# hsinnan75/Kart

Measured on AMD Instinct MI355X. Metric: mapped reads/sec (whole node), 150 bp PE, higher is better.
Workload: dtype u64

## Files before the change

kart_amd/csrc/abi.hip:

```cpp
#include "abi_internal.hpp"
#include <cmath>

#include <algorithm>
#include <atomic>
#include <cstdarg>
#include <cstdio>
#include <cstdlib>
#include <cstring>
#include <memory>
#include <mutex>
#include <string>
#include <thread>
#include <vector>

namespace kg { KG_INTERNAL thread_local KernelTimer *kt_current = nullptr; }

namespace {

thread_local char g_err[512] = "";

}

int kg_fail(int code, const char *fmt, ...)
{
// ... 98 lines not shown
		if (v.seq_len == 0 || v.primary > v.seq_len || (uint64_t)n_words < need)
			return fail(KG_ERR_IO, "%s.bwt is truncated or malformed (%llu words for %llu symbols, need %llu)", prefix, (unsigned long long)n_words,
			            (unsigned long long)v.seq_len, (unsigned long long)need);
	}
	uint64_t sa_intv = 0, sa_len = 0;
	memcpy(&sa_intv, sa.data() + 40, 8);
	memcpy(&sa_len, sa.data() + 48, 8);
	if (sa_intv != 32) return fail(KG_ERR_IO, "%s.sa: unsupported SA interval %llu (expected 32)", prefix, (unsigned long long)sa_intv);
	if (sa_len != v.seq_len) return fail(KG_ERR_IO, "%s: .sa and .bwt disagree on the sequence length", prefix);
	ix->n_sa = (v.seq_len + 32) / 32;
	if ((sa.size() - 56) / 8 < ix->n_sa - 1) return fail(KG_ERR_IO, "%s.sa is truncated", prefix);

	{
		FILE *fp = fopen((pre + ".ann").c_str(), "r");
		if (!fp) return fail(KG_ERR_IO, "cannot read %s.ann", prefix);
		long long l_pac = 0;
		int n_seqs = 0;
		unsigned seed = 0;
		if (fscanf(fp, "%lld%d%u", &l_pac, &n_seqs, &seed) != 3) { fclose(fp); return fail(KG_ERR_IO, "%s.ann: bad header", prefix); }
		ix->l_pac = l_pac;
		int64_t total = 0;
		for (int i = 0; i < n_seqs; ++i) {
			unsigned gi;
			char name[1024];
			long long off;
			int len, n_ambs, ch;
			if (fscanf(fp, "%u%1023s", &gi, name) != 2) { fclose(fp); return fail(KG_ERR_IO, "%s.ann: bad contig record %d", prefix, i); }
			while ((ch = fgetc(fp)) != '\n' && ch != EOF) {}
			if (fscanf(fp, "%lld%d%d", &off, &len, &n_ambs) != 3) { fclose(fp); return fail(KG_ERR_IO, "%s.ann: bad contig record %d", prefix, i); }
			ContigRec c;
			c.name = name;
			c.len = len;
			c.fwd_start = total;
			total += len;
			c.rev_start = 2 * ix->l_pac - total;
			ix->contigs.push_back(c);
		}
		fclose(fp);
		if ((uint64_t)(2 * ix->l_pac) != v.seq_len) return fail(KG_ERR_IO, "%s: .ann l_pac does not match the BWT length", prefix);
	}
	size_t pac_bytes = (size_t)(ix->l_pac / 4 + 1);
	if (pac.size() < pac_bytes) return fail(KG_ERR_IO, "%s.pac is truncated", prefix);
	ix->pac.assign(pac.data(), pac.data() + pac_bytes);

	size_t occ_bytes = n_words * 4 + 128;
	HIP_TRY(hipMalloc((void **)&ix->d_occ, occ_bytes));
	HIP_TRY(hipMemset(ix->d_occ, 0, occ_bytes));
	HIP_TRY(hipMemcpy(ix->d_occ, bwt.data() + 40, n_words * 4, hipMemcpyHostToDevice));
	const uint64_t sa0 = (uint64_t)-1;
	HIP_TRY(hipMalloc((void **)&ix->d_sa, ix->n_sa * 8));
	HIP_TRY(hipMemcpy(ix->d_sa, &sa0, 8, hipMemcpyHostToDevice));
	if (ix->n_sa > 1) HIP_TRY(hipMemcpy(ix->d_sa + 1, sa.data() + 56, (ix->n_sa - 1) * 8, hipMemcpyHostToDevice));
	HIP_TRY(hipMalloc((void **)&ix->d_pac, pac_bytes));
	HIP_TRY(hipMemcpy(ix->d_pac, ix->pac.data(), pac_bytes, hipMemcpyHostToDevice));
	{
		std::vector<std::pair<int64_t, int32_t>> ec;
		for (size_t i = 0; i < ix->contigs.size(); ++i) {
			const ContigRec &c = ix->contigs[i];
			ec.emplace_back(c.fwd_start + c.len - 1, (int32_t)i);
			ec.emplace_back(c.rev_start + c.len - 1, (int32_t)i);
		}
		std::sort(ec.begin(), ec.end());
		std::vector<int64_t> ends;
		std::vector<int32_t> echr;
		for (const std::pair<int64_t, int32_t> &e : ec) { ends.push_back(e.first); echr.push_back(e.second); }
		ix->n_ends = (int)ends.size();
		HIP_TRY(hipMalloc((void **)&ix->d_contig_end, 8 * ends.size() + 8));
		HIP_TRY(hipMemcpy(ix->d_contig_end, ends.data(), 8 * ends.size(), hipMemcpyHostToDevice));
		HIP_TRY(hipMalloc((void **)&ix->d_end_chr, 4 * echr.size() + 8));
		HIP_TRY(hipMemcpy(ix->d_end_chr, echr.data(), 4 * echr.size(), hipMemcpyHostToDevice));
		std::vector<int64_t> tab;
		for (const ContigRec &c : ix->contigs) tab.push_back(c.fwd_start);
		for (const ContigRec &c : ix->contigs) tab.push_back(c.rev_start);
		for (const ContigRec &c : ix->contigs) tab.push_back(c.len);
		HIP_TRY(hipMalloc((void **)&ix->d_chr_tab, 8 * tab.size() + 8));
		HIP_TRY(hipMemcpy(ix->d_chr_tab, tab.data(), 8 * tab.size(), hipMemcpyHostToDevice));
		std::vector<uint8_t> mq((size_t)(kAlnMaxScore + 1) * 6 + (size_t)(kAlnMaxScore + 1) * 8, 0);
		for (int sc = 1; sc <= kAlnMaxScore; ++sc)
			for (int d = 1; d <= 5 && d < sc; ++d) {
				int sub = sc - d;
				int q = (int)(30 * (1 - (float)(sc - sub) / sc) * log(sc) + 0.4999);
				mq[(size_t)sc * 6 + (size_t)d] = (uint8_t)(q > 60 ? 60 : q < 0 ? 0 : q);
			}
		for (int sc = 1; sc < 8; ++sc)
			for (int nd = 1; nd <= kAlnMaxScore; ++nd) {
				int sub = sc + nd;
				int q = (int)(30 * (1 - (float)(sc - sub) / sc) * log(sc) + 0.4999);
				mq[(size_t)(kAlnMaxScore + 1) * 6 + (size_t)sc * (kAlnMaxScore + 1) + (size_t)nd] = (uint8_t)(q > 60 ? 60 : q < 0 ? 0 : q);
			}
		HIP_TRY(hipMalloc((void **)&ix->d_mapq_tab, mq.size()));
		HIP_TRY(hipMemcpy(ix->d_mapq_tab, mq.data(), mq.size(), hipMemcpyHostToDevice));
	}
	ix->device_bytes = occ_bytes + ix->n_sa * 8 + pac_bytes;
	v.occ = ix->d_occ;
	v.sa = ix->d_sa;
	{
		uint64_t n_blocks64 = ((v.seq_len + 127) / 128) * 2;
		size_t plane_bytes = (size_t)n_blocks64 * 64 + 64;
		HIP_TRY(hipMalloc((void **)&ix->d_planes, plane_bytes));
		HIP_TRY(launch_build_planes(ix->d_occ, n_blocks64, ix->d_planes, nullptr));
		HIP_TRY(hipDeviceSynchronize());
		v.planes = ix->d_planes;
		ix->device_bytes += plane_bytes;
	}
	v.planes2 = nullptr;
	v.planes3 = nullptr;
	for (int i = 0; i < 16; ++i) v.t2[i] = 0;
	for (int i = 0; i < 64; ++i) v.t3[i] = 0;
	if (!getenv("KG_NO_PLANES2")) {
		uint64_t n_lines = (v.seq_len + kPlane2Rows - 1) / kPlane2Rows;
		size_t bytes = (size_t)n_lines * 16 * 128;
		uint64_t *t_dev = nullptr;
		if (hipMalloc((void **)&ix->d_planes2, bytes) == hipSuccess) {
			HIP_TRY(hipMalloc((void **)&t_dev, (16 + 64) * 8));
			HIP_TRY(launch_build_planes_k(v, 2, ix->d_planes2, n_lines, t_dev, t_dev + 16, nullptr));
			HIP_TRY(hipMemcpy(v.t2, t_dev, 16 * 8, hipMemcpyDeviceToHost));
			HIP_TRY(hipMemcpy(v.t3, t_dev + 16, 64 * 8, hipMemcpyDeviceToHost));
			HIP_TRY(hipFree(t_dev));
			v.planes2 = ix->d_planes2;
			ix->device_bytes += bytes;
		} else (void)hipGetLastError();
	}
	v.fsa32 = nullptr;
	v.fsa64 = nullptr;
	v.fsa40 = nullptr;
	v.dsa32 = nullptr;
	v.dsa64 = nullptr;
	v.dsa_shift = 0;
	v.text = nullptr;
	{
		size_t text_bytes = (size_t)(v.seq_len / 4 + 1) + 16;
		HIP_TRY(hipMalloc((void **)&ix->d_text, text_bytes));
		HIP_TRY(launch_build_text(ix->d_pac, (uint64_t)ix->l_pac, ix->d_text, text_bytes, nullptr));
		HIP_TRY(hipDeviceSynchronize());
		ix->device_bytes += text_bytes;
	}
	v.qtab32 = nullptr;
	v.qtab64 = nullptr;
	v.qmer = 0;

	const bool dense = sa_mode == KG_SA_DENSE4 || sa_mode == KG_SA_DENSE8;
	const bool wide = sa_mode == KG_SA_FULL40_WIDE;
	const bool compact = sa_mode == KG_SA_FULL40 || wide;
	if (sa_mode == KG_SA_FULL || dense || compact) {
		bool narrow = v.seq_len < 0xFFFFFFFFull && !getenv("KG_FORCE_U64");
		const bool packed = compact && !narrow;
		if (packed && v.seq_len >= (1ull << 40)) return fail(KG_ERR_ARG, "kg_index_load: KG_SA_FULL40 holds texts below 2^40 bases");
		size_t fsa_bytes = packed ? (size_t)(v.seq_len + 1) * 5 + 8 : (size_t)(v.seq_len + 1) * (narrow ? 4 : 8);
		HIP_TRY(hipMalloc(&ix->d_fsa, fsa_bytes));
		uint32_t *f32 = narrow ? (uint32_t *)ix->d_fsa : nullptr;
		uint64_t *f64 = narrow || packed ? nullptr : (uint64_t *)ix->d_fsa;
		uint8_t *f40 = packed ? (uint8_t *)ix->d_fsa : nullptr;
		HIP_TRY(launch_expand_sa(v, ix->n_sa, f32, f64, f40, nullptr));
		HIP_TRY(hipDeviceSynchronize());
		v.fsa32 = f32;
		v.fsa64 = f64;
		v.fsa40 = f40;
		if (!dense) ix->device_bytes += fsa_bytes;
		if (!getenv("KG_NO_DIRECT")) v.text = ix->d_text;
	} else if (sa_mode != KG_SA_SAMPLED) {
		return fail(KG_ERR_ARG, "kg_index_load: unknown sa_mode %d", sa_mode);
	}
	if (!getenv("KG_NO_QTAB")) {
		bool narrow = v.seq_len < 0xFFFFFF00ull && !getenv("KG_FORCE_U64");
		int q = kQmerMin;
		while (q < kQmerMax && ((uint64_t)1 << (2 * q + 1)) <= v.seq_len) q++;
		if (compact && !wide && q > kQmerMin) q--;
		if (const char *env = getenv("KG_QMER")) { int t = atoi(env); if (t >= kQmerMin && t <= kQmerMax) q = t; }
		size_t tab_bytes = ((size_t)1 << (2 * q)) * 8;
		while (hipMalloc(&ix->d_qtab, tab_bytes) != hipSuccess) {
			(void)hipGetLastError();
			ix->d_qtab = nullptr;
			if (q <= kQmerMin) return fail(KG_ERR_NOMEM, "kg_index_load: no device memory for the q-mer table");
			q--;
			tab_bytes >>= 2;
		}
		v.qmer = q;
		HIP_TRY(launch_build_qtab(v, q, narrow ? (uint2 *)ix->d_qtab : nullptr, narrow ? nullptr : (uint64_t *)ix->d_qtab, nullptr));
		HIP_TRY(hipDeviceSynchronize());
		if (narrow) v.qtab32 = (const uint2 *)ix->d_qtab; else v.qtab64 = (const uint64_t *)ix->d_qtab;
		ix->device_bytes += tab_bytes;
	}
	if (dense) {
		const int shift = sa_mode == KG_SA_DENSE4 ? 2 : 3;
		const bool narrow = v.fsa32 != nullptr;
		const uint64_t n_out = (v.seq_len >> shift) + 1;
		const size_t bytes = (size_t)n_out * (narrow ? 4 : 8);
		HIP_TRY(hipMalloc(&ix->d_dsa, bytes));
		HIP_TRY(launch_sample_sa(v.fsa32, v.fsa64, n_out, shift, narrow ? (uint32_t *)ix->d_dsa : nullptr, narrow ? nullptr : (uint64_t *)ix->d_dsa, nullptr));
		HIP_TRY(hipDeviceSynchronize());
		HIP_TRY(hipFree(ix->d_fsa));
		ix->d_fsa = nullptr;
		v.fsa32 = nullptr; v.fsa64 = nullptr;
		if (narrow) v.dsa32 = (const uint32_t *)ix->d_dsa; else v.dsa64 = (const uint64_t *)ix->d_dsa;
		v.dsa_shift = shift;
		ix->device_bytes += bytes;
	}
	if (v.planes2 && !dense && (!compact || wide) && !getenv("KG_NO_PLANES3")) {
		uint64_t n_lines = (v.seq_len + kPlane2Rows - 1) / kPlane2Rows;
		size_t bytes = (size_t)n_lines * 64 * 128, free_b = 0, total_b = 0;
		const size_t reserve = (size_t)48 << 30;
		if (hipMemGetInfo(&free_b, &total_b) == hipSuccess && free_b > bytes + reserve && hipMalloc((void **)&ix->d_planes3, bytes) == hipSuccess) {
			HIP_TRY(launch_build_planes_k(v, 3, ix->d_planes3, n_lines, nullptr, nullptr, nullptr));
			v.planes3 = ix->d_planes3;
			ix->device_bytes += bytes;
		} else (void)hipGetLastError();
	}
	*out = ix.release();
	return KG_OK;
}

void kg_index_destroy(kg_index *ix)
{
	if (!ix) return;
	(void)hipSetDevice(ix->device);
	kgi_frag_release(ix);
	if (ix->d_occ) (void)hipFree(ix->d_occ);
	if (ix->d_planes) (void)hipFree(ix->d_planes);
	if (ix->d_planes2) (void)hipFree(ix->d_planes2);
	if (ix->d_planes3) (void)hipFree(ix->d_planes3);
	if (ix->d_qtab) (void)hipFree(ix->d_qtab);
	for (NwScratch *sc : ix->nw_pool) {
		if (sc->done) { (void)hipEventSynchronize(sc->done); (void)hipEventDestroy(sc->done); }
		if (sc->lists) (void)hipFree(sc->lists);
		if (sc->queue) (void)hipFree(sc->queue);
		if (sc->dir) (void)hipFree(sc->dir);
		if (sc->io) (void)hipFree(sc->io);
		if (sc->io_stream) (void)hipStreamDestroy(sc->io_stream);
		delete sc;
	}
	if (ix->d_sa) (void)hipFree(ix->d_sa);
	if (ix->d_fsa) (void)hipFree(ix->d_fsa);
	if (ix->d_dsa) (void)hipFree(ix->d_dsa);
	if (ix->d_text) (void)hipFree(ix->d_text);
	if (ix->d_pac) (void)hipFree(ix->d_pac);
	if (ix->d_contig_end) (void)hipFree(ix->d_contig_end);
	if (ix->d_end_chr) (void)hipFree(ix->d_end_chr);
	if (ix->d_chr_tab) (void)hipFree(ix->d_chr_tab);
	if (ix->d_mapq_tab) (void)hipFree(ix->d_mapq_tab);
	delete ix;
}

int kg_index_info(const kg_index *ix, kg_index_info_t *info)
{
	if (!ix || !info) return fail(KG_ERR_ARG, "kg_index_info: null argument");
	info->genome_size = ix->l_pac;
	info->seq_len = ix->view.seq_len;
	info->primary = ix->view.primary;
	info->n_contigs = (int32_t)ix->contigs.size();
	int k = 13;
	for (; k < 16; ++k)
		if ((double)(2 * ix->l_pac) < (double)(1ull << (2 * k))) break;
	info->min_seed_len = k;
	info->sa_mode = ix->sa_mode;
	info->device = ix->device;
	info->device_bytes = ix->device_bytes;
	return KG_OK;
}

int kg_index_contig(const kg_index *ix, int i, kg_contig_t *out)
{
	if (!ix || !out || i < 0 || i >= (int)ix->contigs.size()) return fail(KG_ERR_ARG, "kg_index_contig: bad argument");
	const ContigRec &c = ix->contigs[(size_t)i];
	out->name = c.name.c_str();
	out->fwd_start = c.fwd_start;
	out->rev_start = c.rev_start;
	out->len = c.len;
	return KG_OK;
}

int kg_rank_sa_batch(kg_index *ix, const uint64_t *k, int64_t n, uint64_t *occ4, uint64_t *sa_walk, uint64_t *sa_full)
{
	if (!ix || !k || n < 0) return fail(KG_ERR_ARG, "kg_rank_sa_batch: bad argument");
	if (n == 0) return KG_OK;
	HIP_TRY(hipSetDevice(ix->device));
	uint64_t *d = nullptr;
	HIP_TRY(hipMalloc((void **)&d, 8 * (size_t)n * 7));
	uint64_t *d_k = d, *d_occ = d + n, *d_walk = d + 5 * n, *d_full = d + 6 * n;
	hipError_t e = hipMemcpy(d_k, k, 8 * (size_t)n, hipMemcpyHostToDevice);
	if (e == hipSuccess) e = launch_rank_sa(ix->view, d_k, n, occ4 ? d_occ : nullptr, sa_walk ? d_walk : nullptr, sa_full ? d_full : nullptr, nullptr);
	if (e == hipSuccess) e = hipDeviceSynchronize();
	if (e == hipSuccess && occ4) e = hipMemcpy(occ4, d_occ, 32 * (size_t)n, hipMemcpyDeviceToHost);
	if (e == hipSuccess && sa_walk) e = hipMemcpy(sa_walk, d_walk, 8 * (size_t)n, hipMemcpyDeviceToHost);
	if (e == hipSuccess && sa_full) e = hipMemcpy(sa_full, d_full, 8 * (size_t)n, hipMemcpyDeviceToHost);
	(void)hipFree(d);
	if (e != hipSuccess) return fail(KG_ERR_NO_DEVICE, "kg_rank_sa_batch: %s", hipGetErrorString(e));
	return KG_OK;
}

void *kg_host_alloc(size_t bytes)
{
	void *p = nullptr;
	if (hipHostMalloc(&p, bytes ? bytes : 1, hipHostMallocPortable) != hipSuccess) { (void)hipGetLastError(); return nullptr; }
	return p;
}

void kg_host_free(void *p)
{
	if (p) (void)hipHostFree(p);
}

int kg_workspace_create(kg_index *ix, int64_t max_reads, int64_t max_bases, kg_workspace **out)
{
	if (!ix || !out || max_reads <= 0 || max_bases <= 0) return fail(KG_ERR_ARG, "kg_workspace_create: bad argument");
	*out = nullptr;
	HIP_TRY(hipSetDevice(ix->device));
	std::unique_ptr<kg_workspace, void (*)(kg_workspace *)> ws(new kg_workspace(), kg_workspace_destroy);
	ws->ix = ix;
	ws->max_reads = max_reads;
	ws->max_bases = max_bases;
	ws->max_hits = max_bases / 13 + max_bases / 52 + max_reads + (int64_t)ix->n_cu * 32 * 256 + 4096;
	HIP_TRY(hipMalloc((void **)&ws->d_hits, sizeof(Hit) * (size_t)ws->max_hits));
	HIP_TRY(hipMalloc((void **)&ws->d_packed, 8 * (size_t)(max_bases / 16 + 3 * max_reads + 64)));
	HIP_TRY(hipMalloc((void **)&ws->d_seeds_per_read, 4 * (size_t)max_reads));
	HIP_TRY(hipMalloc((void **)&ws->d_ctl, 8 * kCtlWords));
	ws->scan_bytes = scan_temp_bytes(max_reads + 1);
	HIP_TRY(hipMalloc(&ws->d_scan_temp, ws->scan_bytes ? ws->scan_bytes : 256));
	if (getenv("KG_SORT_READS")) {
		ws->sort_bytes = sort_temp_bytes(max_reads);
		HIP_TRY(hipMalloc((void **)&ws->d_sort_keys, 16 * (size_t)max_reads + 64));
		HIP_TRY(hipMalloc(&ws->d_sort_temp, ws->sort_bytes ? ws->sort_bytes : 256));
	}
	HIP_TRY(hipStreamCreateWithFlags(&ws->stream, hipStreamNonBlocking));
	HIP_TRY(hipMemsetAsync(ws->d_ctl, 0, 8 * kCtlWords, ws->stream));
	HIP_TRY(hipHostMalloc((void **)&ws->h_small, 8 * 16, hipHostMallocDefault));
	*out = ws.release();
	return KG_OK;
}

void kg_workspace_destroy(kg_workspace *ws)
{
	if (!ws) return;
	(void)hipSetDevice(ws->ix->device);
	if (ws->stream) { (void)hipStreamSynchronize(ws->stream); (void)hipStreamDestroy(ws->stream); }
	kgi_long_release(ws);
	for (int i = 0; i < kg_workspace::kRing; ++i) {
		if (ws->ring_cands[i]) (void)hipHostFree(ws->ring_cands[i]);
		if (ws->ring_seeds[i]) (void)hipHostFree(ws->ring_seeds[i]);
		if (ws->ring_records[i]) (void)hipHostFree(ws->ring_records[i]);
	}
	void *ptrs[] = {ws->d_sort_keys, ws->d_sort_temp, ws->d_plans, ws->d_tasks, ws->d_aln_cand, ws->d_aln_read, ws->d_spill, ws->d_jobs, ws->d_job_ops, ws->d_job_len, ws->d_chunk_off, ws->d_chunk_paired, ws->d_chunk_stats, ws->d_aln_ctl, ws->d_used, ws->d_cand_off, ws->d_cseed_off, ws->d_dense_cands, ws->d_dense_seeds, ws->d_cands, ws->d_cand_seeds, ws->d_n_cands, ws->d_taken, ws->d_hits, ws->d_packed, ws->d_seeds_per_read, ws->d_ctl, ws->d_scan_temp, ws->d_enc, ws->d_read_off, ws->d_seed_off, ws->d_seeds, ws->d_vr_n, ws->d_vr_off, ws->d_vr_read, ws->d_vr_pos, ws->d_claim, ws->d_step};
	for (void *p : ptrs)
		if (p) (void)hipFree(p);
	if (ws->h_seeds) (void)hipHostFree(ws->h_seeds);
	if (ws->h_small) (void)hipHostFree(ws->h_small);
	if (ws->sync_ev) (void)hipEventDestroy(ws->sync_ev);
	for (hipEvent_t e : ws->ev)
		if (e) (void)hipEventDestroy(e);
	for (int i = 0; i < KT_SLOTS; ++i) {
		for (int j = 0; j < kKtRing; ++j) {
			if (ws->kt.b[i][j]) (void)hipEventDestroy(ws->kt.b[i][j]);
			if (ws->kt.e[i][j]) (void)hipEventDestroy(ws->kt.e[i][j]);
		}
	}
	delete ws;
}

int kg_workspace_counters(kg_workspace *ws, kg_counters_t *out)
{
	if (!ws || !out) return fail(KG_ERR_ARG, "kg_workspace_counters: null argument");
	HIP_TRY(hipSetDevice(ws->ix->device));
	HIP_TRY(hipDeviceSynchronize());
	unsigned long long ctl[kCtlWords];
	HIP_TRY(hipMemcpy(ctl, ws->d_ctl, sizeof(ctl), hipMemcpyDeviceToHost));
	out->searches = ctl[4]; out->lf1 = ctl[5]; out->lf2 = ctl[6]; out->inv = ctl[7];
	out->sa = ctl[8]; out->seeds = ctl[9]; out->bases = ctl[10];
	return KG_OK;
}

int kg_workspace_traffic(kg_workspace *ws, kg_traffic_t *out)
{
	if (!ws || !out) return fail(KG_ERR_ARG, "kg_workspace_traffic: null argument");
	HIP_TRY(hipSetDevice(ws->ix->device));
	HIP_TRY(hipDeviceSynchronize());
	unsigned long long ctl[kCtlWords];
	HIP_TRY(hipMemcpy(ctl, ws->d_ctl, sizeof(ctl), hipMemcpyDeviceToHost));
	out->table_lookups = ctl[17]; out->rank_steps = ctl[18]; out->rank_steps_two_lines = ctl[19];
	out->text_rounds = ctl[20]; out->window_words = ctl[21]; out->rank_steps_two_lines_narrow = ctl[22];
	out->sa_gathers = ctl[8]; out->hits = ctl[1]; out->searches = ctl[4];
	out->sa_entry_bytes = (ws->ix->view.fsa32 ? 4 : ws->ix->view.fsa40 ? 5 : 8);
	out->double_steps = ctl[23]; out->double_steps_two_lines = ctl[24]; out->double_step_bytes = ctl[25]; out->triple_steps = ctl[26];
	return KG_OK;
}

int kg_workspace_set_single_steps(kg_workspace *ws, int enabled)
{
	if (!ws) return fail(KG_ERR_ARG, "kg_workspace_set_single_steps: null workspace");
	ws->single_steps = enabled != 0;
	return KG_OK;
}

int kg_index_selfcheck(kg_index *ix, int64_t samples, uint64_t seed, uint64_t *disagreements)
{
	if (!ix || !disagreements || samples < 0) return fail(KG_ERR_ARG, "kg_index_selfcheck: bad argument");
	*disagreements = 0;
	if (!ix->view.planes2) return fail(KG_ERR_ARG, "kg_index_selfcheck: the index holds no two-step rank structure");
	HIP_TRY(hipSetDevice(ix->device));
	unsigned long long *bad = nullptr;
	HIP_TRY(hipMalloc((void **)&bad, 8));
	HIP_TRY(hipMemset(bad, 0, 8));
	HIP_TRY(hipDeviceSynchronize());
	hipError_t e = launch_planes2_check(ix->view, (uint64_t)samples, seed, bad, nullptr);
	unsigned long long h = 0;
	hipError_t e2 = hipMemcpy(&h, bad, 8, hipMemcpyDeviceToHost);
	(void)hipFree(bad);
	if (e != hipSuccess || e2 != hipSuccess) return fail(KG_ERR_NO_DEVICE, "kg_index_selfcheck: %s", hipGetErrorString(e != hipSuccess ? e : e2));
	*disagreements = h;
	return KG_OK;
}

int kg_workspace_set_profiling(kg_workspace *ws, int enabled)
{
	if (!ws) return fail(KG_ERR_ARG, "kg_workspace_set_profiling: null workspace");
	HIP_TRY(hipSetDevice(ws->ix->device));
	if (enabled && !ws->ev[0])
		for (int i = 0; i < 5; ++i) HIP_TRY(hipEventCreate(&ws->ev[i]));
	if (enabled && !ws->kt.b[0][0])
		for (int i = 0; i < KT_SLOTS; ++i)
			for (int j = 0; j < kKtRing; ++j) { HIP_TRY(hipEventCreate(&ws->kt.b[i][j])); HIP_TRY(hipEventCreate(&ws->kt.e[i][j])); }
	ws->profiling = enabled != 0;
	return KG_OK;
}

int kg_workspace_kernel_ms(kg_workspace *ws, float ms[4])
{
	if (!ws || !ms) return fail(KG_ERR_ARG, "kg_workspace_kernel_ms: null argument");
	if (!ws->profiling || !ws->ev[0]) return fail(KG_ERR_ARG, "kg_workspace_kernel_ms: profiling is not enabled");
	HIP_TRY(hipSetDevice(ws->ix->device));
	HIP_TRY(hipEventSynchronize(ws->ev[4]));
	for (int i = 0; i < 4; ++i) HIP_TRY(hipEventElapsedTime(&ms[i], ws->ev[i], ws->ev[i + 1]));
	return KG_OK;
}

int64_t kg_workspace_overflow(kg_workspace *ws)
{
	if (!ws) return -1;
	if (hipSetDevice(ws->ix->device) != hipSuccess || hipDeviceSynchronize() != hipSuccess) return -1;
	unsigned long long v = 0;
	if (hipMemcpy(&v, ws->d_ctl + 11, 8, hipMemcpyDeviceToHost) != hipSuccess) return -1;
	return (int64_t)v;
}

int64_t kg_workspace_segment_fallbacks(kg_workspace *ws)
{
	return ws ? ws->segment_fallbacks : -1;
}

static int check_seed_args(kg_workspace *ws, int mode, int min_seed_len, int occ_thr, int64_t n_reads, int64_t n_bases)
{
	if (!ws) return fail(KG_ERR_ARG, "kg_seed_batch: null workspace");
	if ((mode & ~KG_INPUT_ASCII) != KG_MODE_FAST && (mode & ~KG_INPUT_ASCII) != KG_MODE_SENSITIVE) return fail(KG_ERR_ARG, "kg_seed_batch: unknown mode %d", mode);
	if (min_seed_len < 13 || min_seed_len > 16) return fail(KG_ERR_ARG, "kg_seed_batch: min_seed_len %d outside 13..16", min_seed_len);
	if (occ_thr < 1 || occ_thr > 1000000) return fail(KG_ERR_ARG, "kg_seed_batch: occ_thr %d out of range", occ_thr);
	if (n_reads < 0 || n_reads > ws->max_reads) return fail(KG_ERR_CAPACITY, "kg_seed_batch: %lld reads exceed the workspace (%lld)", (long long)n_reads, (long long)ws->max_reads);
	if (n_bases < 0 || n_bases > ws->max_bases) return fail(KG_ERR_CAPACITY, "kg_seed_batch: %lld bases exceed the workspace (%lld)", (long long)n_bases, (long long)ws->max_bases);
	return KG_OK;
}

int kg_seed_batch_device(kg_workspace *ws, int mode, int min_seed_len, int occ_thr, const uint8_t *d_enc_bases,
                         const int64_t *d_read_offsets, int64_t n_reads, int64_t n_bases, int64_t *d_seed_offsets,
                         kg_seed *d_seeds, int64_t seed_capacity, void *stream)
{
	int rc = check_seed_args(ws, mode, min_seed_len, occ_thr, n_reads, n_bases);
	if (rc != KG_OK) return rc;
	if (!d_read_offsets || !d_seed_offsets || (n_bases > 0 && !d_enc_bases) || (seed_capacity > 0 && !d_seeds) || seed_capacity < 0)
		return fail(KG_ERR_ARG, "kg_seed_batch_device: null buffer");
	HIP_TRY(hipSetDevice(ws->ix->device));
	hipStream_t st = (hipStream_t)stream;
	if (n_reads == 0) {
		HIP_TRY(hipMemsetAsync(d_seed_offsets, 0, 8, st));
		return KG_OK;
	}
	SeedArgs a;
	a.ix = ws->ix->view;
	a.enc = d_enc_bases;
	a.read_off = d_read_offsets;
	a.n_reads = n_reads;
	a.n_bases = n_bases;
	a.mode = mode & ~KG_INPUT_ASCII;
	a.ascii = (mode & KG_INPUT_ASCII) ? 1 : 0;
	a.min_seed_len = min_seed_len;
	a.occ_thr = occ_thr;
	a.packed = ws->d_packed;
	a.single_steps = ws->single_steps ? 1 : 0;
	a.read_order = nullptr; a.sort_keys = ws->d_sort_keys; a.sort_temp = ws->d_sort_temp; a.sort_temp_bytes = ws->sort_bytes;
	a.hits = ws->d_hits;
	a.max_hits = ws->max_hits;
	a.seeds_per_read = ws->d_seeds_per_read;
	a.read_queue = ws->d_ctl + 0;
	a.hit_count = ws->d_ctl + 1;
	a.locate_queue = ws->d_ctl + 2;
	a.counters = ws->d_ctl + 4;
	a.traffic = ws->d_ctl + 17;
	a.seed_off = d_seed_offsets;
	a.seeds = d_seeds;
	a.seed_capacity = seed_capacity;
	a.read_len = nullptr; a.n_seg = 0; a.seg_stride = 0;
	for (int64_t &x : a.seg_prefix) x = 0;
	const bool no_segments = getenv("KG_NO_SEGMENTS") != nullptr;
	const int seg_len = getenv("KG_SEG_LEN") ? std::max(128, atoi(getenv("KG_SEG_LEN"))) : 512;
	ws->last_segmented = false;
	if (a.mode == KG_MODE_SENSITIVE && !no_segments && ws->segments_off_batches == 0 && ws->group_segments == 0 && n_bases >= 4 * (int64_t)seg_len * n_reads) {
		ws->last_segmented = true;
		if (!ws->d_vr_n) {
			ws->vr_capacity = ws->max_bases / 128 + ws->max_reads + 64;
			HIP_TRY(hipMalloc((void **)&ws->d_vr_n, 4 * (size_t)(ws->max_reads + 2)));
			HIP_TRY(hipMalloc((void **)&ws->d_vr_off, 8 * (size_t)(ws->max_reads + 2)));
			HIP_TRY(hipMalloc((void **)&ws->d_vr_read, 4 * (size_t)ws->vr_capacity));
			HIP_TRY(hipMalloc((void **)&ws->d_vr_pos, 4 * (size_t)ws->vr_capacity));
			HIP_TRY(hipMalloc((void **)&ws->d_claim, 4 * (size_t)((ws->max_bases >> 5) + ws->max_reads + 64)));
			HIP_TRY(hipMalloc((void **)&ws->d_step, (size_t)ws->max_bases + 64));
		}
		a.seg_len = seg_len;
		a.vr_read = ws->d_vr_read; a.vr_pos = ws->d_vr_pos;
		a.vr_total = reinterpret_cast<const unsigned long long *>(ws->d_vr_off + n_reads);
		a.claim = ws->d_claim; a.step = ws->d_step;
		HIP_TRY(launch_seed_segments(a, ws->d_vr_n, ws->d_vr_off, ws->d_vr_read, ws->d_vr_pos, ws->d_scan_temp, ws->scan_bytes, ws->ix->n_cu, st));
	}
	if (ws->group_segments > 0) {
		a.read_len = ws->group_read_len;
		a.n_seg = ws->group_segments;
		a.seg_stride = ws->group_stride;
		for (int i = 0; i <= a.n_seg; ++i) a.seg_prefix[i] = ws->group_prefix[i];
	}
	HIP_TRY(launch_seed_batch(a, ws->d_scan_temp, ws->scan_bytes, ws->ix->n_cu, st, ws->profiling ? ws->ev : nullptr));
	return KG_OK;
}

hipError_t kgi_sync(kg_workspace *ws)
{
	static const bool spin = getenv("KG_SPIN_SYNC") != nullptr;
	if (spin) return hipStreamSynchronize(ws->stream);
	if (!ws->sync_ev) {
		hipError_t e = hipEventCreateWithFlags(&ws->sync_ev, hipEventBlockingSync | hipEventDisableTiming);
		if (e != hipSuccess) return e;
	}
	hipError_t e = hipEventRecord(ws->sync_ev, ws->stream);
	if (e != hipSuccess) return e;
	return hipEventSynchronize(ws->sync_ev);
}

int kgi_seed_resident(kg_workspace *ws, int mode, int min_seed_len, int occ_thr, int64_t n_reads, int64_t n_bases, int64_t *total_out)
{
	int rc = check_seed_args(ws, mode, min_seed_len, occ_thr, n_reads, n_bases);
	if (rc != KG_OK) return rc;
	int64_t want = std::max<int64_t>(ws->seed_capacity, 8 * std::max(n_reads, ws->max_reads) + 1024);
	int64_t total = 0;
	bool retried_plain = false;
	for (int attempt = 0; attempt < 2; ++attempt) {
		if (want > ws->seed_capacity) {
			if (ws->d_seeds) HIP_TRY(hipFree(ws->d_seeds));
			ws->d_seeds = nullptr;
			HIP_TRY(hipMalloc((void **)&ws->d_seeds, sizeof(kg_seed) * (size_t)want));
			ws->seed_capacity = want;
		}
		rc = kg_seed_batch_device(ws, mode, min_seed_len, occ_thr, ws->d_enc, ws->d_read_off, n_reads, n_bases,
		                          ws->d_seed_off, ws->d_seeds, ws->seed_capacity, ws->stream);
		if (rc != KG_OK) return rc;
		unsigned long long *h = ws->h_small;
		HIP_TRY(hipMemcpyAsync(&h[0], ws->d_seed_off + n_reads, 8, hipMemcpyDeviceToHost, ws->stream));
		HIP_TRY(hipMemcpyAsync(&h[1], ws->d_ctl + 11, 8, hipMemcpyDeviceToHost, ws->stream));
		HIP_TRY(kgi_sync(ws));
		if (h[1] == (~0ull >> 1)) {
			if (ws->last_segmented && !retried_plain) {
				retried_plain = true;
				ws->segments_off_batches = 17;
				ws->segment_fallbacks++;
				--attempt;
				continue;
			}
			return fail(KG_ERR_CAPACITY, "kg_seed_batch: the hit list of the workspace overflowed");
		}
		total = (int64_t)h[0];
		if (total <= ws->seed_capacity) break;
		want = total;
		if (attempt == 1) return fail(KG_ERR_CAPACITY, "kg_seed_batch: seed buffer overflow persisted");
	}
	if (ws->segments_off_batches > 0) ws->segments_off_batches--;
	ws->last_reads = n_reads;
	ws->last_seeds = total;
	ws->last_cands = -1;
	ws->last_ascii = (mode & KG_INPUT_ASCII) != 0;
	*total_out = total;
	return KG_OK;
}

int kgi_seed_group(kg_workspace *ws, int mode, int min_seed_len, int occ_thr, int n_seg, int64_t stride, const int64_t *counts, int64_t *seed_base)
{
	if (n_seg < 1 || n_seg > kMaxSeedSegments || stride < 1 || (int64_t)n_seg * stride > ws->max_reads) return fail(KG_ERR_ARG, "kgi_seed_group: %d segments of %lld slots do not fit the group's workspace", n_seg, (long long)stride);
	ws->group_segments = n_seg;
	ws->group_stride = stride;
	ws->group_prefix[0] = 0;
	for (int i = 0; i < n_seg; ++i) {
		if (counts[i] < 0 || counts[i] > stride) return fail(KG_ERR_ARG, "kgi_seed_group: segment %d holds %lld reads, its slots are %lld", i, (long long)counts[i], (long long)stride);
		ws->group_prefix[i + 1] = ws->group_prefix[i] + counts[i];
	}
	const int64_t n_slots = (int64_t)n_seg * stride;
	int64_t total = 0;
	int rc = kgi_seed_resident(ws, mode, min_seed_len, occ_thr, n_slots, ws->max_bases, &total);
	if (rc != KG_OK) return rc;
	unsigned long long *h = ws->h_small;
	for (int i = 0; i < n_seg; ++i) HIP_TRY(hipMemcpyAsync(&h[2 + i], ws->d_seed_off + (int64_t)i * stride, 8, hipMemcpyDeviceToHost, ws->stream));
	HIP_TRY(kgi_sync(ws));
	for (int i = 0; i < n_seg; ++i) seed_base[i] = (int64_t)h[2 + i];
	seed_base[n_seg] = total;
	return KG_OK;
}

int kg_seed_batch(kg_workspace *ws, int mode, int min_seed_len, int occ_thr, const uint8_t *enc_bases,
                  const int64_t *read_offsets, int64_t n_reads, int64_t *seed_offsets, const kg_seed **seeds)
{
	if (!ws || !read_offsets || !seed_offsets) return fail(KG_ERR_ARG, "kg_seed_batch: null argument");
	if (seeds) *seeds = nullptr;
	int64_t n_bases = n_reads > 0 ? read_offsets[n_reads] - read_offsets[0] : 0;
	if (n_reads > 0 && read_offsets[0] != 0) return fail(KG_ERR_ARG, "kg_seed_batch: read_offsets[0] must be 0");
	int rc = check_seed_args(ws, mode, min_seed_len, occ_thr, n_reads, n_bases);
	if (rc != KG_OK) return rc;
	if (n_reads == 0) { seed_offsets[0] = 0; return KG_OK; }
	HIP_TRY(hipSetDevice(ws->ix->device));
	if (!ws->d_enc) {
		HIP_TRY(hipMalloc((void **)&ws->d_enc, (size_t)ws->max_bases + 64));
		HIP_TRY(hipMalloc((void **)&ws->d_read_off, 8 * (size_t)(ws->max_reads + 1)));
		HIP_TRY(hipMalloc((void **)&ws->d_seed_off, 8 * (size_t)(ws->max_reads + 1)));
	}
	HIP_TRY(hipMemcpyAsync(ws->d_enc, enc_bases, (size_t)n_bases, hipMemcpyHostToDevice, ws->stream));
	HIP_TRY(hipMemcpyAsync(ws->d_read_off, read_offsets, 8 * (size_t)(n_reads + 1), hipMemcpyHostToDevice, ws->stream));
	int64_t total = 0;
	rc = kgi_seed_resident(ws, mode, min_seed_len, occ_thr, n_reads, n_bases, &total);
	if (rc != KG_OK) return rc;
	HIP_TRY(hipMemcpyAsync(seed_offsets, ws->d_seed_off, 8 * (size_t)(n_reads + 1), hipMemcpyDeviceToHost, ws->stream));
	HIP_TRY(kgi_sync(ws));
	if (!seeds) return KG_OK;
	if (total > ws->h_seed_capacity) {
		if (ws->h_seeds) HIP_TRY(hipHostFree(ws->h_seeds));
		ws->h_seeds = nullptr;
		int64_t cap = std::max<int64_t>(total, ws->seed_capacity);
		HIP_TRY(hipHostMalloc((void **)&ws->h_seeds, sizeof(kg_seed) * (size_t)cap, hipHostMallocDefault));
// ... 481 lines not shown
```

kart_amd/csrc/abi_internal.hpp:

```cpp
#pragma once
#include "seed_kernels.hpp"
#include "align_kernels.hpp"

#include <mutex>
#include <string>
#include <vector>

#define KG_INTERNAL __attribute__((visibility("hidden")))
KG_INTERNAL int kg_fail(int code, const char *fmt, ...);

#define HIP_TRY(expr)                                                                                     \
	do {                                                                                                  \
		hipError_t e_ = (expr);                                                                           \
		if (e_ != hipSuccess) return kg_fail(e_ == hipErrorOutOfMemory ? KG_ERR_NOMEM : KG_ERR_NO_DEVICE, \
		                                     "%s: %s", #expr, hipGetErrorString(e_));                     \
	} while (0)

using namespace kg;

struct ContigRec {
	std::string name;
	int64_t fwd_start, rev_start, len;
};

struct NwScratch {
	int32_t *lists = nullptr;
	size_t list_words = 0;
	unsigned long long *queue = nullptr;
	uint32_t *dir = nullptr;
	size_t dir_words = 0;
	hipEvent_t done = nullptr;
	bool busy = false;
	bool pending = false;
	hipStream_t last_stream = nullptr;
	char *io = nullptr;
	size_t io_bytes = 0;
	bool io_busy = false;
	hipStream_t io_stream = nullptr;
};

struct kg_index {
	std::mutex nw_mu;
	std::vector<NwScratch *> nw_pool;
	int device = 0;
	int n_cu = 256;
	int sa_mode = KG_SA_SAMPLED;
	FmView view{};
	int64_t l_pac = 0;
	uint64_t n_sa = 0;
	std::vector<ContigRec> contigs;
	std::vector<uint8_t> pac;
	uint32_t *d_occ = nullptr;
	uint4 *d_planes = nullptr;
	uint4 *d_planes2 = nullptr;
	uint4 *d_planes3 = nullptr;
	void *d_qtab = nullptr;
	uint64_t *d_sa = nullptr;
	void *d_fsa = nullptr;
	void *d_dsa = nullptr;
	uint8_t *d_text = nullptr;
	uint8_t *d_pac = nullptr;
	int64_t *d_contig_end = nullptr;
	int n_ends = 0;
	int32_t *d_end_chr = nullptr;
	int64_t *d_chr_tab = nullptr;
	uint8_t *d_mapq_tab = nullptr;
	uint64_t device_bytes = 0;
};

struct kg_workspace {
	kg_index *ix = nullptr;
	int64_t max_reads = 0, max_bases = 0, max_hits = 0;
	Hit *d_hits = nullptr;
	uint64_t *d_packed = nullptr;
	int32_t *d_seeds_per_read = nullptr;
	unsigned long long *d_ctl = nullptr;
	void *d_scan_temp = nullptr;
	size_t scan_bytes = 0;
	uint32_t *d_sort_keys = nullptr;
	bool single_steps = false;
	void *d_sort_temp = nullptr;
	size_t sort_bytes = 0;
	uint8_t *d_enc = nullptr;
	int64_t *d_read_off = nullptr;
	int64_t *d_seed_off = nullptr;
	kg_seed *d_seeds = nullptr;
	int64_t seed_capacity = 0;
	int64_t last_reads = 0, last_seeds = 0;
	int group_segments = 0;
	bool last_segmented = false;
	int segments_off_batches = 0;
	int64_t segment_fallbacks = 0;
	int64_t group_stride = 0, group_prefix[kMaxSeedSegments + 1] = {0};
	int32_t *group_read_len = nullptr;
	bool enc_borrowed = false;
	kg_candidate *d_cands = nullptr;
	kg_seed *d_cand_seeds = nullptr;
	int32_t *d_n_cands = nullptr;
	uint8_t *d_taken = nullptr;
	int32_t *d_used = nullptr;
	int64_t *d_cand_off = nullptr, *d_cseed_off = nullptr;
	kg_candidate *d_dense_cands = nullptr, *h_cands = nullptr;
	kg_seed *d_dense_seeds = nullptr, *h_cand_seeds = nullptr;
	int64_t h_cand_capacity = 0;
	static constexpr int kRing = 4;
	kg_candidate *ring_cands[kRing] = {nullptr, nullptr, nullptr, nullptr};
	kg_seed *ring_seeds[kRing] = {nullptr, nullptr, nullptr, nullptr};
	int64_t ring_cand_capacity[kRing] = {0, 0, 0, 0};
	kg_aln_record *ring_records[kRing] = {nullptr, nullptr, nullptr, nullptr};
	int64_t ring_record_capacity[kRing] = {0, 0, 0, 0};
	int ring_at = 0, ring_rec_at = 0;
	int64_t cand_capacity = 0, ncand_capacity = 0;
	kg_seed *h_seeds = nullptr;
	int64_t h_seed_capacity = 0;
	int64_t last_cands = -1;
	int64_t last_cand_seeds = 0;
	bool last_pacbio = false;
	void *lr = nullptr;
	int32_t *d_vr_n = nullptr, *d_vr_read = nullptr, *d_vr_pos = nullptr;
	int64_t *d_vr_off = nullptr;
	uint32_t *d_claim = nullptr;
	uint8_t *d_step = nullptr;
	int64_t vr_capacity = 0;
	bool last_ascii = false;
	void *d_aln_cand = nullptr;
	int64_t aln_cand_capacity = 0;
	void *d_aln_read = nullptr;
	int64_t aln_read_capacity = 0;
	kg_aln_record *h_records = nullptr;
	AlnSpill *d_spill = nullptr;
	NwJobDesc *d_jobs = nullptr;
	uint8_t *d_job_ops = nullptr;
	int32_t *d_job_len = nullptr;
	int64_t spill_capacity = 0, job_capacity = 0, ops_capacity = 0;
	void *d_plans = nullptr;
	void *d_tasks = nullptr;
	int64_t task_capacity = 0;
	int64_t *d_chunk_off = nullptr;
	uint8_t *d_chunk_paired = nullptr;
	kg_chunk_stats *d_chunk_stats = nullptr;
	int chunk_capacity = 0;
	unsigned long long *d_aln_ctl = nullptr;
	hipStream_t stream = nullptr;
	hipEvent_t sync_ev = nullptr;
	unsigned long long *h_small = nullptr;
	bool profiling = false;
	hipEvent_t ev[5] = {nullptr, nullptr, nullptr, nullptr, nullptr};
	KernelTimer kt;
};


extern "C" {
KG_INTERNAL hipError_t kgi_sync(kg_workspace *ws);
KG_INTERNAL int kgi_seed_resident(kg_workspace *ws, int mode, int min_seed_len, int occ_thr, int64_t n_reads, int64_t n_bases, int64_t *total_out);
KG_INTERNAL int kgi_seed_group(kg_workspace *ws, int mode, int min_seed_len, int occ_thr, int n_seg, int64_t stride, const int64_t *counts, int64_t *seed_base);
KG_INTERNAL int kgi_chain_resident(kg_workspace *ws, int pacbio, int max_gaps, int64_t totals[2]);
KG_INTERNAL int kgi_nw_launch(kg_index *ix, NwArgs &a, int64_t max_len, hipStream_t st);
KG_INTERNAL void kgi_long_release(kg_workspace *ws);
KG_INTERNAL void kgi_frag_release(kg_index *ix);
KG_INTERNAL int kgi_align_resident(kg_workspace *ws, const int64_t *chunk_off, const uint8_t *chunk_paired, int n_chunks, int est_distance, int max_insert,
                       int max_gaps, int multi_hit, int unset_flag, int64_t host_record_capacity, AlnArgs &a);
}
```

kart_amd/csrc/abi_stream.hip:

```cpp
#include "abi_internal.hpp"
#include "stream_kernels.hpp"

#include <algorithm>
#include <chrono>
#include <condition_variable>
#include <cstdlib>
#include <cstring>
#include <memory>

#define fail kg_fail

namespace {

struct Lane {
	kg_workspace *ws = nullptr;
	uint8_t *d_text[2] = {nullptr, nullptr};
	int32_t *d_tile[2] = {nullptr, nullptr};
	uint32_t *d_line_end[2] = {nullptr, nullptr};
	uint32_t *d_rec[2] = {nullptr, nullptr};
	uint64_t *d_line_acc[2] = {nullptr, nullptr};
	uint32_t *d_rec_line[2] = {nullptr, nullptr};
	int64_t *d_meta = nullptr;
	int32_t *d_read_len = nullptr;
	void *d_scan = nullptr;
	size_t scan_bytes = 0;
	int32_t *d_sam_len = nullptr, *d_host_list = nullptr;
	int64_t *d_sam_off = nullptr;
	unsigned long long *d_sam_ctl = nullptr;
	uint8_t *d_sam = nullptr;
	int64_t d_sam_capacity = 0;
	char *h_text[2] = {nullptr, nullptr};
	int64_t *h_meta = nullptr;
	char *h_sam = nullptr;
	int64_t h_sam_capacity = 0;
	int64_t *h_sam_off = nullptr, *h_cand_off = nullptr;
	int32_t *h_host_list = nullptr;
	uint32_t *h_rec_hdr[2] = {nullptr, nullptr};
	kg_aln_record *h_records = nullptr;
	int64_t record_capacity = 0;
	kg_chunk_stats *h_chunk_stats = nullptr;
	int64_t chunk_capacity = 0;
	kg_candidate *h_cands = nullptr;
	kg_seed *h_cand_seeds = nullptr;
	int64_t h_cand_capacity = 0;
	unsigned long long *h_ctl = nullptr;
	int64_t mapped_reads = 0;
	const kg_aln_record *d_records = nullptr;
	kg_stream_window win{};
	kg_stream_parsed parsed{};
	bool have_batch = false;
	bool fasta = false;
	hipEvent_t ev[8] = {nullptr, nullptr, nullptr, nullptr, nullptr, nullptr, nullptr, nullptr};
	hipEvent_t ev_parsed = nullptr;
};

struct SeedGroup {
	int first = 0, size = 0;
	int64_t stride = 0, seg_bases = 0;
	kg_workspace *ws = nullptr;
	unsigned long long *h_ctl = nullptr;
	std::mutex mu;
	std::condition_variable cv;
	int64_t round = 0;
	int arrived = 0;
	bool present[kMaxSeedSegments] = {false};
	int absent_rounds[kMaxSeedSegments] = {0};
	int64_t n_reads[kMaxSeedSegments] = {0};
	int rc = KG_OK;
	int64_t seed_base[kMaxSeedSegments + 1] = {0};
	bool aborted = false;
	int order[kMaxSeedSegments] = {0};
	int n_order = 0, turn = 0;
};

struct GroupTurn {
	SeedGroup *sg = nullptr;
	bool held = false;
	bool acquire(SeedGroup &g, int j)
	{
		sg = &g;
		std::unique_lock<std::mutex> lk(g.mu);
		g.cv.wait(lk, [&]() { return g.aborted || (g.turn < g.n_order && g.order[g.turn] == j); });
		held = !g.aborted;
		return held;
	}
	void release()
	{
		if (!held) return;
		held = false;
		std::lock_guard<std::mutex> lk(sg->mu);
		sg->turn++;
		sg->cv.notify_all();
	}
	~GroupTurn() { release(); }
};

}

struct kg_stream {
	kg_index *ix = nullptr;
	kg_stream_config cfg{};
	int64_t text_capacity = 0, line_capacity = 0, rec_capacity = 0;
	std::vector<Lane> lanes;
	std::vector<std::unique_ptr<SeedGroup>> groups;
	uint8_t *d_chr_names = nullptr;
	int32_t *d_chr_name_off = nullptr;
	int min_seed_len = 13;
	int format = KG_STREAM_FORMAT_SAM;
	int input = KG_STREAM_INPUT_FASTQ;
	bool fasta_sized = false;
	std::mutex mu;
	kg_stream_timing_t total{};
};

namespace {

void free_lane(Lane &l)
{
	if (l.ws && l.ws->enc_borrowed) l.ws->d_enc = nullptr;
	if (l.ev_parsed) (void)hipEventDestroy(l.ev_parsed);
	if (l.ws) kg_workspace_destroy(l.ws);
	for (int f = 0; f < 2; ++f) {
		if (l.d_text[f]) (void)hipFree(l.d_text[f]);
		if (l.d_tile[f]) (void)hipFree(l.d_tile[f]);
		if (l.d_line_end[f]) (void)hipFree(l.d_line_end[f]);
		if (l.d_rec[f]) (void)hipFree(l.d_rec[f]);
		if (l.d_line_acc[f]) (void)hipFree(l.d_line_acc[f]);
		if (l.d_rec_line[f]) (void)hipFree(l.d_rec_line[f]);
		if (l.h_text[f]) (void)hipHostFree(l.h_text[f]);
		if (l.h_rec_hdr[f]) (void)hipHostFree(l.h_rec_hdr[f]);
	}
	for (void *p : {(void *)l.d_meta, (void *)l.d_read_len, l.d_scan, (void *)l.d_sam_len, (void *)l.d_host_list, (void *)l.d_sam_off, (void *)l.d_sam_ctl, (void *)l.d_sam})
		if (p) (void)hipFree(p);
	for (void *p : {(void *)l.h_meta, (void *)l.h_sam, (void *)l.h_sam_off, (void *)l.h_cand_off, (void *)l.h_host_list, (void *)l.h_records, (void *)l.h_chunk_stats,
	                (void *)l.h_cands, (void *)l.h_cand_seeds, (void *)l.h_ctl})
		if (p) (void)hipHostFree(p);
	for (hipEvent_t e : l.ev)
		if (e) (void)hipEventDestroy(e);
	l = Lane();
}

FqWindow window_of(const kg_stream *s, const Lane &l, int f)
{
	FqWindow w;
	w.text = l.d_text[f];
	w.begin = l.win.begin[f]; w.end = l.win.end[f]; w.eof = l.win.eof[f];
	w.tile_lines = l.d_tile[f];
	w.line_end = l.d_line_end[f];
	w.line_capacity = s->line_capacity;
	uint32_t *r = l.d_rec[f];
	const size_t c = (size_t)s->rec_capacity;
	w.rec_hdr = r; w.rec_name = r + c; w.rec_seq = r + 2 * c; w.rec_qual = r + 3 * c;
	w.rec_rlen = (int32_t *)(r + 4 * c); w.rec_qlen = (int32_t *)(r + 5 * c);
	w.rec_capacity = s->rec_capacity;
	w.line_acc = l.d_line_acc[f]; w.rec_line = l.d_rec_line[f];
	return w;
}

int64_t out_capacity(const kg_stream_config &cfg, int format)
{
	return 2 * cfg.max_window + (format == KG_STREAM_FORMAT_BAM ? 144 : 64) * cfg.max_reads + 4096;
}

float elapsed(hipEvent_t a, hipEvent_t b)
{
	float ms = 0;
	if (hipEventElapsedTime(&ms, a, b) != hipSuccess) { (void)hipGetLastError(); return 0; }
	return ms;
}

}

extern "C" {

int kg_stream_open(kg_index *ix, const kg_stream_config *cfg, kg_stream **out)
{
	if (!ix || !cfg || !out) return fail(KG_ERR_ARG, "kg_stream_open: null argument");
	*out = nullptr;
	if (cfg->lanes < 1 || cfg->lanes > 16 || cfg->max_reads < 2 || cfg->max_window < 4096 || cfg->max_window > 0xF0000000ll)
		return fail(KG_ERR_ARG, "kg_stream_open: bad configuration (%d lanes, %lld reads, %lld bytes per window)", cfg->lanes, (long long)cfg->max_reads, (long long)cfg->max_window);
	const int group = cfg->seed_group > 1 ? cfg->seed_group : 0;
	if (group && (group > kMaxSeedSegments || cfg->lanes % group != 0))
		return fail(KG_ERR_ARG, "kg_stream_open: seed_group %d must divide the %d lanes and be at most %d", group, cfg->lanes, kMaxSeedSegments);
	if (!ix->d_text) return fail(KG_ERR_ARG, "kg_stream_open: the index holds no text");
	HIP_TRY(hipSetDevice(ix->device));
	std::unique_ptr<kg_stream, void (*)(kg_stream *)> s(new kg_stream(), kg_stream_close);
	s->ix = ix;
	s->cfg = *cfg;
	s->text_capacity = (cfg->max_window + 4096 + 255) & ~255ll;
	s->line_capacity = cfg->max_window / 16 + 4096;
	s->rec_capacity = s->line_capacity / 4 + 1;
	{
		kg_index_info_t info;
		kg_index_info(ix, &info);
		s->min_seed_len = info.min_seed_len;
		std::vector<int32_t> off{0};
		std::string names;
		for (const ContigRec &c : ix->contigs) { names += c.name; off.push_back((int32_t)names.size()); }
		HIP_TRY(hipMalloc((void **)&s->d_chr_names, names.size() + 16));
		HIP_TRY(hipMalloc((void **)&s->d_chr_name_off, 4 * off.size()));
		HIP_TRY(hipMemcpy(s->d_chr_names, names.data(), names.size(), hipMemcpyHostToDevice));
		HIP_TRY(hipMemcpy(s->d_chr_name_off, off.data(), 4 * off.size(), hipMemcpyHostToDevice));
	}
	s->lanes.resize((size_t)cfg->lanes);
	const int64_t n = cfg->max_reads;
	const int64_t seg_bases = (cfg->max_window + 4096 + 64 + 255) & ~255ll;
	for (int g = 0; group && g < cfg->lanes / group; ++g) {
		s->groups.push_back(std::unique_ptr<SeedGroup>(new SeedGroup()));
		SeedGroup *sg = s->groups.back().get();
		sg->first = g * group; sg->size = group;
		sg->stride = n + 8; sg->seg_bases = seg_bases;
		int rc = kg_workspace_create(ix, sg->stride * group, seg_bases * group, &sg->ws);
		if (rc != KG_OK) return rc;
		kg_workspace *gw = sg->ws;
		HIP_TRY(hipMalloc((void **)&gw->d_enc, (size_t)gw->max_bases + 64));
		HIP_TRY(hipMalloc((void **)&gw->d_read_off, 8 * (size_t)(gw->max_reads + 1)));
		HIP_TRY(hipMalloc((void **)&gw->d_seed_off, 8 * (size_t)(gw->max_reads + 1)));
		HIP_TRY(hipMalloc((void **)&gw->group_read_len, 4 * (size_t)(gw->max_reads + 1)));
		HIP_TRY(hipMemsetAsync(gw->d_enc, 'N', (size_t)gw->max_bases + 64, gw->stream));
		HIP_TRY(hipMemsetAsync(gw->d_read_off, 0, 8 * (size_t)(gw->max_reads + 1), gw->stream));
		HIP_TRY(hipMemsetAsync(gw->group_read_len, 0, 4 * (size_t)(gw->max_reads + 1), gw->stream));
		HIP_TRY(hipStreamSynchronize(gw->stream));
		HIP_TRY(hipHostMalloc((void **)&sg->h_ctl, 8 * kCtlWords, hipHostMallocDefault));
		(void)kg_workspace_set_profiling(gw, 1);
	}
	for (size_t li = 0; li < s->lanes.size(); ++li) {
		Lane &l = s->lanes[li];
		int rc = kg_workspace_create(ix, n + 8, cfg->max_window + 4096, &l.ws);
		if (rc != KG_OK) return rc;
		kg_workspace *ws = l.ws;
		if (group) {
			SeedGroup &sg = *s->groups[li / (size_t)group];
			ws->d_enc = sg.ws->d_enc + (int64_t)(li % (size_t)group) * sg.seg_bases;
			ws->enc_borrowed = true;
			HIP_TRY(hipEventCreateWithFlags(&l.ev_parsed, hipEventDisableTiming));
		} else
		HIP_TRY(hipMalloc((void **)&ws->d_enc, (size_t)ws->max_bases + 64));
		HIP_TRY(hipMalloc((void **)&ws->d_read_off, 8 * (size_t)(ws->max_reads + 1)));
		HIP_TRY(hipMalloc((void **)&ws->d_seed_off, 8 * (size_t)(ws->max_reads + 1)));
		(void)kg_workspace_set_profiling(ws, 1);
		const int64_t n_tiles = s->text_capacity / kFqTile + 2;
		for (int f = 0; f < 2; ++f) {
			HIP_TRY(hipMalloc((void **)&l.d_text[f], (size_t)s->text_capacity));
			HIP_TRY(hipMalloc((void **)&l.d_tile[f], 4 * (size_t)(n_tiles + 1)));
			HIP_TRY(hipMalloc((void **)&l.d_line_end[f], 4 * (size_t)s->line_capacity));
			HIP_TRY(hipMalloc((void **)&l.d_rec[f], 4 * 6 * (size_t)s->rec_capacity));
			HIP_TRY(hipHostMalloc((void **)&l.h_text[f], (size_t)s->text_capacity, hipHostMallocDefault));
			HIP_TRY(hipHostMalloc((void **)&l.h_rec_hdr[f], 4 * (size_t)(n + 8), hipHostMallocDefault));
		}
		HIP_TRY(hipMalloc((void **)&l.d_meta, 8 * FQM_WORDS));
		HIP_TRY(hipMalloc((void **)&l.d_read_len, 4 * (size_t)(n + 8)));
		l.scan_bytes = fq_scan_temp_bytes(std::max<int64_t>(n + 8, n_tiles + 1));
		HIP_TRY(hipMalloc(&l.d_scan, l.scan_bytes ? l.scan_bytes : 256));
		HIP_TRY(hipMalloc((void **)&l.d_sam_len, 4 * (size_t)(n + 8)));
		HIP_TRY(hipMalloc((void **)&l.d_host_list, 4 * (size_t)(n + 8)));
		HIP_TRY(hipMalloc((void **)&l.d_sam_off, 8 * (size_t)(n + 8)));
		HIP_TRY(hipMalloc((void **)&l.d_sam_ctl, 8 * 4));
		HIP_TRY(hipHostMalloc((void **)&l.h_meta, 8 * (FQM_WORDS + 24), hipHostMallocDefault));
		HIP_TRY(hipHostMalloc((void **)&l.h_sam_off, 8 * (size_t)(n + 8), hipHostMallocDefault));
		HIP_TRY(hipHostMalloc((void **)&l.h_cand_off, 8 * (size_t)(n + 8), hipHostMallocDefault));
		HIP_TRY(hipHostMalloc((void **)&l.h_host_list, 4 * (size_t)(n + 8), hipHostMallocDefault));
		HIP_TRY(hipHostMalloc((void **)&l.h_ctl, 8 * kCtlWords, hipHostMallocDefault));
		l.d_sam_capacity = out_capacity(*cfg, KG_STREAM_FORMAT_SAM);
		HIP_TRY(hipMalloc((void **)&l.d_sam, (size_t)l.d_sam_capacity));
		l.h_sam_capacity = l.d_sam_capacity;
		HIP_TRY(hipHostMalloc((void **)&l.h_sam, (size_t)l.h_sam_capacity, hipHostMallocDefault));
		l.record_capacity = n + n / 4 + 4096;
		HIP_TRY(hipHostMalloc((void **)&l.h_records, sizeof(kg_aln_record) * (size_t)l.record_capacity, hipHostMallocDefault));
		for (hipEvent_t &e : l.ev) HIP_TRY(hipEventCreate(&e));
	}
	HIP_TRY(hipDeviceSynchronize());
	*out = s.release();
	return KG_OK;
}

void kg_stream_close(kg_stream *s)
{
	if (!s) return;
	(void)hipSetDevice(s->ix->device);
	for (Lane &l : s->lanes) free_lane(l);
	for (std::unique_ptr<SeedGroup> &sg : s->groups) {
		if (sg->ws && sg->ws->group_read_len) { (void)hipFree(sg->ws->group_read_len); sg->ws->group_read_len = nullptr; }
		if (sg->ws) kg_workspace_destroy(sg->ws);
		if (sg->h_ctl) (void)hipHostFree(sg->h_ctl);
	}
	if (s->d_chr_names) (void)hipFree(s->d_chr_names);
	if (s->d_chr_name_off) (void)hipFree(s->d_chr_name_off);
	delete s;
}

int kg_stream_set_format(kg_stream *s, int format)
{
	if (!s) return fail(KG_ERR_ARG, "kg_stream_set_format: null stream");
	if (format != KG_STREAM_FORMAT_SAM && format != KG_STREAM_FORMAT_BAM) return fail(KG_ERR_ARG, "kg_stream_set_format: unknown format %d (KG_STREAM_FORMAT_SAM or KG_STREAM_FORMAT_BAM)", format);
	HIP_TRY(hipSetDevice(s->ix->device));
	const int64_t want = out_capacity(s->cfg, format);
	for (Lane &l : s->lanes) {
		if (l.d_sam_capacity < want) {
			HIP_TRY(hipStreamSynchronize(l.ws->stream));
			HIP_TRY(hipFree(l.d_sam)); l.d_sam = nullptr; l.d_sam_capacity = 0;
			HIP_TRY(hipMalloc((void **)&l.d_sam, (size_t)want));
			l.d_sam_capacity = want;
		}
		if (l.h_sam_capacity < want) {
			HIP_TRY(hipStreamSynchronize(l.ws->stream));
			HIP_TRY(hipHostFree(l.h_sam)); l.h_sam = nullptr; l.h_sam_capacity = 0;
			HIP_TRY(hipHostMalloc((void **)&l.h_sam, (size_t)want, hipHostMallocDefault));
			l.h_sam_capacity = want;
		}
	}
	s->format = format;
	return KG_OK;
}

int kg_stream_set_input(kg_stream *s, int input)
{
	if (!s) return fail(KG_ERR_ARG, "kg_stream_set_input: null stream");
	if (input != KG_STREAM_INPUT_FASTQ && input != KG_STREAM_INPUT_FASTA) return fail(KG_ERR_ARG, "kg_stream_set_input: unknown input %d (KG_STREAM_INPUT_FASTQ or KG_STREAM_INPUT_FASTA)", input);
	HIP_TRY(hipSetDevice(s->ix->device));
	if (input == KG_STREAM_INPUT_FASTA) {
		const size_t want_scan = fa_scan_temp_bytes(s->line_capacity);
		const int64_t rec_capacity = s->line_capacity / 2 + 1;
		for (Lane &l : s->lanes) {
			if (s->fasta_sized) break;
			HIP_TRY(hipStreamSynchronize(l.ws->stream));
			for (int f = 0; f < 2; ++f) {
				uint32_t *wider = nullptr;
				HIP_TRY(hipMalloc((void **)&wider, 4 * 6 * (size_t)rec_capacity));
				(void)hipFree(l.d_rec[f]);
				l.d_rec[f] = wider;
				if (!l.d_line_acc[f]) HIP_TRY(hipMalloc((void **)&l.d_line_acc[f], 8 * (size_t)(s->line_capacity + 1)));
				if (!l.d_rec_line[f]) HIP_TRY(hipMalloc((void **)&l.d_rec_line[f], 4 * (size_t)(rec_capacity + 1)));
				HIP_TRY(hipMemset(l.d_line_acc[f], 0, 8 * (size_t)(s->line_capacity + 1)));
				HIP_TRY(hipMemset(l.d_rec_line[f], 0, 4 * (size_t)(rec_capacity + 1)));
			}
			if (l.scan_bytes < want_scan) {
				HIP_TRY(hipStreamSynchronize(l.ws->stream));
				HIP_TRY(hipFree(l.d_scan)); l.d_scan = nullptr; l.scan_bytes = 0;
				HIP_TRY(hipMalloc(&l.d_scan, want_scan));
				l.scan_bytes = want_scan;
			}
		}
	}
	if (input == KG_STREAM_INPUT_FASTA && !s->fasta_sized) { s->rec_capacity = s->line_capacity / 2 + 1; s->fasta_sized = true; }
	s->input = input;
	return KG_OK;
}

char *kg_stream_staging(kg_stream *s, int lane, int file, int64_t *capacity)
{
	if (!s || lane < 0 || lane >= (int)s->lanes.size() || file < 0 || file > 1) return nullptr;
	if (capacity) *capacity = s->cfg.max_window;
	return s->lanes[(size_t)lane].h_text[file];
}

int kg_stream_upload(kg_stream *s, int lane, int file, int64_t from, int64_t to)
{
	if (!s || lane < 0 || lane >= (int)s->lanes.size() || file < 0 || file > 1) return fail(KG_ERR_ARG, "kg_stream_upload: bad argument");
	if (from < 0 || to < from || to > s->cfg.max_window) return fail(KG_ERR_ARG, "kg_stream_upload: range [%lld, %lld) outside the staging buffer", (long long)from, (long long)to);
	if (to == from) return KG_OK;
	Lane &l = s->lanes[(size_t)lane];
	HIP_TRY(hipSetDevice(s->ix->device));
	HIP_TRY(hipMemcpyAsync(l.d_text[file] + from, l.h_text[file] + from, (size_t)(to - from), hipMemcpyHostToDevice, l.ws->stream));
	return KG_OK;
}

int kg_stream_parse(kg_stream *s, int lane, const kg_stream_window *w, kg_stream_parsed *out)
{
	if (!s || !w || !out || lane < 0 || lane >= (int)s->lanes.size()) return fail(KG_ERR_ARG, "kg_stream_parse: bad argument");
	Lane &l = s->lanes[(size_t)lane];
	const int nf = w->two_files ? 2 : 1;
	for (int f = 0; f < nf; ++f)
		if (w->begin[f] < 0 || w->end[f] < w->begin[f] || w->end[f] > s->cfg.max_window) return fail(KG_ERR_ARG, "kg_stream_parse: window %d outside the staging buffer", f);
	if (w->chunk_reads < 2 || (w->chunk_reads & 1) || w->want_reads < w->chunk_reads || w->want_reads > s->cfg.max_reads || w->want_reads % w->chunk_reads)
		return fail(KG_ERR_ARG, "kg_stream_parse: want_reads must be a multiple of chunk_reads (an even number) within the stream's batch size");
	HIP_TRY(hipSetDevice(s->ix->device));
	l.win = *w;
	l.have_batch = false;
	l.fasta = s->input == KG_STREAM_INPUT_FASTA;
	kg_workspace *ws = l.ws;
	FqArgs a;
	a.w[0] = window_of(s, l, 0);
	a.w[1] = window_of(s, l, 1);
	if (!w->two_files) { a.w[1].begin = a.w[1].end = 0; a.w[1].eof = 1; }
	a.two_files = w->two_files ? 1 : 0;
	a.paired = w->paired ? 1 : 0;
	a.chunk_reads = w->chunk_reads;
	a.fasta = s->input == KG_STREAM_INPUT_FASTA ? 1 : 0;
	a.gz_lines = w->gz_lines ? 1 : 0;
	a.max_reads = s->cfg.max_reads;
	a.want_reads = w->want_reads;
	a.meta = l.d_meta;
	a.read_len = l.d_read_len;
	a.read_off = ws->d_read_off;
	a.enc = ws->d_enc;
	a.n_reads = 0;
	hipStream_t st = ws->stream;
	KtUse kt_use(ws->profiling ? &ws->kt : nullptr);
	HIP_TRY(hipEventRecord(l.ev[0], st));
	HIP_TRY(launch_fq_parse(a, l.d_scan, l.scan_bytes, s->ix->n_cu, st));
	HIP_TRY(hipMemcpyAsync(l.h_meta, l.d_meta, 8 * FQM_WORDS, hipMemcpyDeviceToHost, st));
	HIP_TRY(kgi_sync(ws));
	kg_stream_parsed &p = l.parsed;
	p.n_reads = l.h_meta[FQM_READS]; p.n_chunks = l.h_meta[FQM_CHUNKS]; p.n_bases = l.h_meta[FQM_BASES];
	p.used[0] = l.h_meta[FQM_USED0]; p.used[1] = w->two_files ? l.h_meta[FQM_USED1] : 0;
	p.stop = (int32_t)l.h_meta[FQM_STOP]; p.done = (int32_t)l.h_meta[FQM_DONE];
	if (p.n_bases > ws->max_bases) return fail(KG_ERR_CAPACITY, "kg_stream_parse: %lld bases exceed the lane's workspace (%lld)", (long long)p.n_bases, (long long)ws->max_bases);
	if (p.n_reads > 0) {
		a.n_reads = p.n_reads;
		HIP_TRY(launch_fq_materialise(a, s->ix->n_cu, st));
		const int64_t r0 = w->two_files ? p.n_reads / 2 : p.n_reads;
		HIP_TRY(hipMemcpyAsync(l.h_rec_hdr[0], a.w[0].rec_hdr, 4 * (size_t)r0, hipMemcpyDeviceToHost, st));
		if (w->two_files) HIP_TRY(hipMemcpyAsync(l.h_rec_hdr[1], a.w[1].rec_hdr, 4 * (size_t)r0, hipMemcpyDeviceToHost, st));
	}
	if (!s->groups.empty() && p.n_reads > 0) {
		SeedGroup &sg = *s->groups[(size_t)lane / (size_t)s->cfg.seed_group];
		const int j = lane - sg.first;
		HIP_TRY(launch_group_publish(ws->d_read_off, p.n_reads, sg.stride, (int64_t)j * sg.seg_bases, sg.ws->d_read_off + (int64_t)j * sg.stride,
		                             sg.ws->group_read_len + (int64_t)j * sg.stride, s->ix->n_cu, st));
		HIP_TRY(hipEventRecord(l.ev_parsed, st));
	}
	HIP_TRY(hipEventRecord(l.ev[1], st));
	l.have_batch = p.n_reads > 0;
	*out = p;
	return KG_OK;
}

static int group_seed(kg_stream *s, int lane, int64_t n, int64_t n_bases, int64_t *n_seeds, bool *was_leader, float *search_ms, double *useful_bytes)
{
	SeedGroup &sg = *s->groups[(size_t)lane / (size_t)s->cfg.seed_group];
	Lane &l = s->lanes[(size_t)lane];
	const int j = lane - sg.first;
	*was_leader = false;
	std::unique_lock<std::mutex> lk(sg.mu);
	if (sg.aborted) return fail(KG_ERR_ARG, "kg_stream_map: the stream's seeding groups were aborted");
	if (sg.absent_rounds[j] < 0) return fail(KG_ERR_ARG, "kg_stream_map: lane %d was declared absent until further notice (kg_stream_group_absent) and arrives with a batch", lane);
	if (!sg.cv.wait_for(lk, std::chrono::seconds(600), [&]() { return sg.absent_rounds[j] == 0 || sg.aborted; })) {
		sg.aborted = true;
		sg.cv.notify_all();
		return fail(KG_ERR_ARG, "kg_stream_map: lane %d waited 600 s for the round it declared itself absent from", lane);
	}
	if (sg.aborted) return fail(KG_ERR_ARG, "kg_stream_map: the stream's seeding groups were aborted");
	const int64_t my_round = sg.round;
	sg.present[j] = true;
	sg.n_reads[j] = n;
	sg.arrived++;
	auto complete = [&]() {
		int accounted = sg.arrived;
		for (int i = 0; i < sg.size; ++i) accounted += (!sg.present[i] && sg.absent_rounds[i] != 0) ? 1 : 0;
		return accounted >= sg.size;
	};
	auto run_round = [&]() {
		kg_workspace *gw = sg.ws;
		int64_t counts[kMaxSeedSegments];
		int rc = KG_OK;
		for (int i = 0; i < sg.size && rc == KG_OK; ++i) {
			counts[i] = sg.present[i] ? sg.n_reads[i] : 0;
			if (hipStreamWaitEvent(gw->stream, s->lanes[(size_t)(sg.first + i)].ev_parsed, 0) != hipSuccess) rc = fail(KG_ERR_NO_DEVICE, "kg_stream_map: hipStreamWaitEvent");
		}
		if (rc == KG_OK) rc = kgi_seed_group(gw, KG_MODE_FAST | KG_INPUT_ASCII, s->min_seed_len, KG_OCC_THR_DEFAULT, sg.size, sg.stride, counts, sg.seed_base);
		if (rc == KG_OK && (hipMemcpyAsync(sg.h_ctl, gw->d_ctl, 8 * kCtlWords, hipMemcpyDeviceToHost, gw->stream) != hipSuccess || kgi_sync(gw) != hipSuccess))
			rc = fail(KG_ERR_NO_DEVICE, "kg_stream_map: reading the group's counters back");
		sg.rc = rc;
		sg.n_order = 0; sg.turn = 0;
		for (int i = 0; i < sg.size; ++i)
			if (sg.present[i]) sg.order[sg.n_order++] = i;
		for (int i = 0; i < sg.size; ++i) {
			sg.present[i] = false;
			if (sg.absent_rounds[i] > 0) sg.absent_rounds[i]--;
		}
		sg.arrived = 0;
		sg.round++;
		sg.cv.notify_all();
	};
	const std::chrono::steady_clock::time_point give_up = std::chrono::steady_clock::now() + std::chrono::seconds(600);
	auto leave = [&]() {
		if (sg.round == my_round && sg.present[j]) { sg.present[j] = false; sg.arrived--; }
	};
	for (;;) {
		if (sg.aborted) { leave(); return fail(KG_ERR_ARG, "kg_stream_map: the stream's seeding groups were aborted"); }
		if (sg.round != my_round) break;
		if (complete()) {
			run_round();
			*was_leader = true;
			if (sg.rc == KG_OK) {
				kg_workspace *gw = sg.ws;
				*search_ms = gw->profiling && gw->ev[0] ? elapsed(gw->ev[0], gw->ev[1]) : 0;
				const unsigned long long *c = sg.h_ctl;
				const double sa_bytes = s->ix->view.fsa32 ? 4.0 : 8.0;
				const int64_t reads = gw->group_prefix[sg.size];
				*useful_bytes = 8.0 * (double)c[17] + 32.0 * (double)c[18] + (double)c[25] + sa_bytes * (double)c[8] + 48.0 * (double)c[20] + 8.0 * (double)c[21] + 20.0 * (double)reads + 32.0 * (double)c[1];
			}
			break;
		}
		if (sg.cv.wait_until(lk, give_up) == std::cv_status::timeout) {
			sg.aborted = true;
			sg.cv.notify_all();
			leave();
			return fail(KG_ERR_ARG, "kg_stream_map: lane %d waited 600 s for the other lanes of its seeding group (a lane without a batch must call kg_stream_group_absent)", lane);
		}
	}
	if (sg.rc != KG_OK) return sg.rc;
	const int64_t first = sg.seed_base[j], count = (j + 1 < sg.size ? sg.seed_base[j + 1] : sg.seed_base[sg.size]) - first;
	lk.unlock();
	kg_workspace *ws = l.ws, *gw = sg.ws;
	if (count > ws->seed_capacity) {
		if (ws->d_seeds) HIP_TRY(hipFree(ws->d_seeds));
		ws->d_seeds = nullptr;
		const int64_t want = std::max<int64_t>(count + count / 4, 8 * ws->max_reads + 1024);
		HIP_TRY(hipMalloc((void **)&ws->d_seeds, sizeof(kg_seed) * (size_t)want));
		ws->seed_capacity = want;
	}
	HIP_TRY(launch_group_rebase(gw->d_seed_off + (int64_t)j * sg.stride, n, first, ws->d_seed_off, s->ix->n_cu, ws->stream));
	if (count > 0) HIP_TRY(hipMemcpyAsync(ws->d_seeds, gw->d_seeds + first, sizeof(kg_seed) * (size_t)count, hipMemcpyDeviceToDevice, ws->stream));
	ws->last_reads = n; ws->last_seeds = count; ws->last_cands = -1; ws->last_ascii = true;
	(void)n_bases;
	*n_seeds = count;
	return KG_OK;
}

int kg_stream_map(kg_stream *s, int lane, const kg_stream_params *prm, kg_stream_result *out)
{
	if (!s || !prm || !out || lane < 0 || lane >= (int)s->lanes.size()) return fail(KG_ERR_ARG, "kg_stream_map: bad argument");
	Lane &l = s->lanes[(size_t)lane];
	if (!l.have_batch) return fail(KG_ERR_ARG, "kg_stream_map: no parsed batch in lane %d (kg_stream_parse first)", lane);
	memset(out, 0, sizeof(*out));
	kg_index *ix = s->ix;
	kg_workspace *ws = l.ws;
	hipStream_t st = ws->stream;
	HIP_TRY(hipSetDevice(ix->device));
	KtUse kt_use(ws->profiling ? &ws->kt : nullptr);
	const int64_t n = l.parsed.n_reads;
	const int n_chunks = (int)l.parsed.n_chunks;
	int64_t n_seeds = 0, totals[2] = {0, 0};
	const bool grouped = !s->groups.empty();
	bool group_leader = false;
	float group_search_ms = 0;
	double group_useful = 0;
	int rc;
	GroupTurn turn;
	if (grouped) {
		rc = group_seed(s, lane, n, l.parsed.n_bases, &n_seeds, &group_leader, &group_search_ms, &group_useful);
		static const bool no_turns = getenv("KG_GROUP_NO_TURNS") != nullptr;
		SeedGroup &sg = *s->groups[(size_t)lane / (size_t)s->cfg.seed_group];
		if (rc == KG_OK && !no_turns && !turn.acquire(sg, lane - sg.first)) rc = fail(KG_ERR_ARG, "kg_stream_map: the stream's seeding groups were aborted");
		if (rc != KG_OK) {
			std::lock_guard<std::mutex> lk(sg.mu);
			sg.aborted = true;
			sg.cv.notify_all();
		}
	} else rc = kgi_seed_resident(ws, KG_MODE_FAST | KG_INPUT_ASCII, s->min_seed_len, KG_OCC_THR_DEFAULT, n, l.parsed.n_bases, &n_seeds);
	if (rc != KG_OK) return rc;
	if (!grouped) HIP_TRY(hipMemcpyAsync(l.h_ctl, ws->d_ctl, 8 * kCtlWords, hipMemcpyDeviceToHost, st));
	HIP_TRY(hipEventRecord(l.ev[2], st));
	rc = kgi_chain_resident(ws, 0, prm->max_gaps, totals);
	if (rc != KG_OK) return rc;
	HIP_TRY(hipEventRecord(l.ev[3], st));
	std::vector<int64_t> chunk_off((size_t)n_chunks + 1);
	std::vector<uint8_t> chunk_paired((size_t)n_chunks, (uint8_t)(l.win.paired ? 1 : 0));
	for (int c = 0; c <= n_chunks; ++c) chunk_off[(size_t)c] = std::min<int64_t>(n, (int64_t)c * l.win.chunk_reads);
	if (n_chunks > l.chunk_capacity) {
		if (l.h_chunk_stats) HIP_TRY(hipHostFree(l.h_chunk_stats));
		l.h_chunk_stats = nullptr;
		l.chunk_capacity = n_chunks + n_chunks / 2 + 64;
		HIP_TRY(hipHostMalloc((void **)&l.h_chunk_stats, sizeof(kg_chunk_stats) * (size_t)l.chunk_capacity, hipHostMallocDefault));
	}
	AlnArgs a;
	rc = kgi_align_resident(ws, chunk_off.data(), chunk_paired.data(), n_chunks, prm->est_distance, prm->max_insert, prm->max_gaps, prm->multi_hit,
	                        prm->unset_flag, l.record_capacity, a);
	if (rc != KG_OK) return rc;
	HIP_TRY(hipEventRecord(l.ev[4], st));
	SamArgs q;
	q.w[0] = window_of(s, l, 0); q.w[1] = window_of(s, l, 1);
	q.two_files = l.win.two_files ? 1 : 0; q.paired = l.win.paired ? 1 : 0;
	q.fasta = l.fasta ? 1 : 0;
	q.enc = ws->d_enc; q.read_off = ws->d_read_off; q.n_reads = n;
	q.records = a.records;
	q.chr_names = s->d_chr_names; q.chr_name_off = s->d_chr_name_off;
	q.sam_len = l.d_sam_len; q.sam_off = l.d_sam_off; q.sam = l.d_sam; q.sam_capacity = l.d_sam_capacity;
	q.host_list = l.d_host_list; q.ctl = l.d_sam_ctl;
	const bool bam = s->format == KG_STREAM_FORMAT_BAM;
	HIP_TRY(bam ? launch_bam_size(q, l.d_scan, l.scan_bytes, ix->n_cu, st) : launch_sam_size(q, l.d_scan, l.scan_bytes, ix->n_cu, st));
	int64_t *tot = l.h_meta + FQM_WORDS;
	HIP_TRY(hipMemcpyAsync(&tot[0], l.d_sam_off + n, 8, hipMemcpyDeviceToHost, st));
	HIP_TRY(hipMemcpyAsync(&tot[1], l.d_sam_ctl, 8, hipMemcpyDeviceToHost, st));
	HIP_TRY(hipMemcpyAsync(&tot[3], ws->d_aln_ctl + 7, 8, hipMemcpyDeviceToHost, st));
	HIP_TRY(kgi_sync(ws));
	const int64_t sam_bytes = tot[0], n_host = tot[1];
	const int64_t extra = prm->multi_hit ? std::min<int64_t>(tot[3], a.extra_capacity) : 0;
	if (sam_bytes > l.d_sam_capacity) {
		HIP_TRY(hipFree(l.d_sam)); l.d_sam = nullptr;
		l.d_sam_capacity = sam_bytes + sam_bytes / 4;
		HIP_TRY(hipMalloc((void **)&l.d_sam, (size_t)l.d_sam_capacity));
		q.sam = l.d_sam; q.sam_capacity = l.d_sam_capacity;
	}
	if (sam_bytes > l.h_sam_capacity) {
		HIP_TRY(hipHostFree(l.h_sam)); l.h_sam = nullptr;
		l.h_sam_capacity = sam_bytes + sam_bytes / 4;
		HIP_TRY(hipHostMalloc((void **)&l.h_sam, (size_t)l.h_sam_capacity, hipHostMallocDefault));
	}
	const int64_t cand_need = std::max(totals[0], totals[1]);
	if (cand_need > l.h_cand_capacity) {
		if (l.h_cands) HIP_TRY(hipHostFree(l.h_cands));
		if (l.h_cand_seeds) HIP_TRY(hipHostFree(l.h_cand_seeds));
		l.h_cands = nullptr; l.h_cand_seeds = nullptr;
		l.h_cand_capacity = std::max<int64_t>(cand_need + cand_need / 4 + 1024, 3 * s->cfg.max_reads);
		HIP_TRY(hipHostMalloc((void **)&l.h_cands, sizeof(kg_candidate) * (size_t)l.h_cand_capacity, hipHostMallocDefault));
		HIP_TRY(hipHostMalloc((void **)&l.h_cand_seeds, sizeof(kg_seed) * (size_t)l.h_cand_capacity, hipHostMallocDefault));
	}
	HIP_TRY(bam ? launch_bam_format(q, ix->n_cu, st) : launch_sam_format(q, ix->n_cu, st));
	const bool checksum = getenv("KG_STREAM_CHECKSUM") != nullptr;
	if (checksum) HIP_TRY(launch_sam_checksum(q, ix->n_cu, st));
	HIP_TRY(hipEventRecord(l.ev[5], st));
	static const bool turn_early = getenv("KG_GROUP_TURN_EARLY") != nullptr;
	if (turn_early) turn.release();
	if (sam_bytes > 0) HIP_TRY(hipMemcpyAsync(l.h_sam, l.d_sam, (size_t)sam_bytes, hipMemcpyDeviceToHost, st));
	HIP_TRY(hipMemcpyAsync(l.h_sam_off, l.d_sam_off, 8 * (size_t)(n + 1), hipMemcpyDeviceToHost, st));
	const bool all = prm->fetch_all != 0;
	l.mapped_reads = n; l.d_records = a.records;
	if (all) HIP_TRY(hipMemcpyAsync(l.h_records, a.records, sizeof(kg_aln_record) * (size_t)(n + extra), hipMemcpyDeviceToHost, st));
	else if (extra > 0) HIP_TRY(hipMemcpyAsync(l.h_records + n, a.records + n, sizeof(kg_aln_record) * (size_t)extra, hipMemcpyDeviceToHost, st));
	HIP_TRY(hipMemcpyAsync(l.h_chunk_stats, ws->d_chunk_stats, sizeof(kg_chunk_stats) * (size_t)n_chunks, hipMemcpyDeviceToHost, st));
	if (all) HIP_TRY(hipMemcpyAsync(l.h_cand_off, ws->d_cand_off, 8 * (size_t)(n + 1), hipMemcpyDeviceToHost, st));
	if (n_host > 0) HIP_TRY(hipMemcpyAsync(l.h_host_list, l.d_host_list, 4 * (size_t)n_host, hipMemcpyDeviceToHost, st));
	if (all && totals[0] > 0) HIP_TRY(hipMemcpyAsync(l.h_cands, ws->d_dense_cands, sizeof(kg_candidate) * (size_t)totals[0], hipMemcpyDeviceToHost, st));
	if (all && totals[1] > 0) HIP_TRY(hipMemcpyAsync(l.h_cand_seeds, ws->d_dense_seeds, sizeof(kg_seed) * (size_t)totals[1], hipMemcpyDeviceToHost, st));
	HIP_TRY(hipMemcpyAsync(&tot[2], l.d_sam_ctl + 1, 8, hipMemcpyDeviceToHost, st));
	HIP_TRY(hipMemcpyAsync(&tot[8], ws->d_aln_ctl, 8 * 7, hipMemcpyDeviceToHost, st));
	HIP_TRY(hipMemcpyAsync(&tot[15], ws->d_aln_ctl + 32, 8, hipMemcpyDeviceToHost, st));
	tot[16] = tot[17] = 0;
	if (checksum) HIP_TRY(hipMemcpyAsync(&tot[16], l.d_sam_ctl + 2, 16, hipMemcpyDeviceToHost, st));
	HIP_TRY(hipMemcpyAsync(&tot[14], ws->d_aln_ctl + 36, 8, hipMemcpyDeviceToHost, st));
	HIP_TRY(hipEventRecord(l.ev[6], st));
	HIP_TRY(kgi_sync(ws));
	if (tot[2] != 0) return fail(KG_ERR_NO_DEVICE, "kg_stream_map: %lld records were formatted to a size other than the one announced", (long long)tot[2]);
	std::sort(l.h_host_list, l.h_host_list + n_host);
	out->n_reads = n; out->n_chunks = n_chunks;
	out->sam = l.h_sam; out->sam_bytes = sam_bytes; out->sam_off = l.h_sam_off;
	out->records = l.h_records; out->n_records = n + extra;
	out->chunk_stats = l.h_chunk_stats;
	out->host_reads = l.h_host_list; out->n_host_reads = n_host;
	out->cand_off = l.h_cand_off; out->cands = l.h_cands; out->cand_seeds = l.h_cand_seeds;
	out->rec_start[0] = l.h_rec_hdr[0]; out->rec_start[1] = l.win.two_files ? l.h_rec_hdr[1] : nullptr;
	l.have_batch = false;
	{
		float sk = 0;
		if (!grouped && ws->profiling && ws->ev[0]) sk = elapsed(ws->ev[0], ws->ev[1]);
		const unsigned long long *c = l.h_ctl;
		const double sa_bytes = ix->view.fsa32 ? 4.0 : 8.0;
		double useful = grouped ? 0.0 : 8.0 * (double)c[17] + 32.0 * (double)c[18] + (double)c[25] + sa_bytes * (double)c[8] + 48.0 * (double)c[20] + 8.0 * (double)c[21] + 20.0 * (double)n + 32.0 * (double)c[1];
		if (grouped && group_leader) { sk = group_search_ms; useful = group_useful; }
		std::lock_guard<std::mutex> lk(s->mu);
		kg_stream_timing_t &t = s->total;
		t.batches += 1; t.reads += n;
		t.parse_ms += elapsed(l.ev[0], l.ev[1]); t.seed_ms += elapsed(l.ev[1], l.ev[2]); t.chain_ms += elapsed(l.ev[2], l.ev[3]);
		t.align_ms += elapsed(l.ev[3], l.ev[4]); t.format_ms += elapsed(l.ev[4], l.ev[5]); t.copy_ms += elapsed(l.ev[5], l.ev[6]);
		t.search_kernel_ms += sk; t.search_kernel_launches += (!grouped || group_leader) ? 1 : 0; t.search_useful_bytes += useful;
		t.text_in_bytes += (double)((l.parsed.used[0] - l.win.begin[0]) + (l.win.two_files ? l.parsed.used[1] - l.win.begin[1] : 0));
		t.text_out_bytes += (double)sam_bytes;
		t.candidates += (double)totals[0]; t.candidate_seeds += (double)totals[1];
		for (int i = 0; i < 8; ++i) t.aln_counts[i] += (double)tot[8 + i];
		t.text_checksum[0] += (double)(uint64_t)tot[16]; t.text_checksum[1] += (double)(uint64_t)tot[17];
		for (int i = 0; i < KT_SLOTS; ++i) {
			const int used = ws->kt.used[i];
			if (!used) continue;
			ws->kt.used[i] = 0;
			for (int j = 0; j < used; ++j) t.kernel_ms[i] += elapsed(ws->kt.b[i][j], ws->kt.e[i][j]);
			t.kernel_launches[i] += used;
		}
	}
	return KG_OK;
}

int kg_stream_group_absent(kg_stream *s, int lane, int rounds)
{
	if (!s || lane < 0 || lane >= (int)s->lanes.size()) return fail(KG_ERR_ARG, "kg_stream_group_absent: bad argument");
	if (s->groups.empty()) return KG_OK;
	SeedGroup &sg = *s->groups[(size_t)lane / (size_t)s->cfg.seed_group];
	const int j = lane - sg.first;
	std::unique_lock<std::mutex> lk(sg.mu);
	if (sg.present[j]) return fail(KG_ERR_ARG, "kg_stream_group_absent: lane %d is inside a round", lane);
	if (rounds != 0) {
		Lane &l = s->lanes[(size_t)lane];
		HIP_TRY(hipSetDevice(s->ix->device));
		HIP_TRY(launch_group_publish(l.ws->d_read_off, 0, sg.stride, (int64_t)j * sg.seg_bases, sg.ws->d_read_off + (int64_t)j * sg.stride, sg.ws->group_read_len + (int64_t)j * sg.stride,
		                             s->ix->n_cu, l.ws->stream));
		HIP_TRY(hipEventRecord(l.ev_parsed, l.ws->stream));
	}
	sg.absent_rounds[j] = rounds;
	if (rounds == 0) sg.aborted = false;
	int accounted = sg.arrived;
	for (int i = 0; i < sg.size; ++i) accounted += (!sg.present[i] && sg.absent_rounds[i] != 0) ? 1 : 0;
	if (rounds != 0 && sg.arrived > 0 && accounted >= sg.size) sg.cv.notify_all();
	if (rounds > 0 && sg.arrived == 0 && accounted >= sg.size) {
		for (int i = 0; i < sg.size; ++i)
			if (sg.absent_rounds[i] > 0) sg.absent_rounds[i]--;
		sg.round++;
		sg.cv.notify_all();
	}
	return KG_OK;
}

int kg_stream_group_abort(kg_stream *s)
{
	if (!s) return fail(KG_ERR_ARG, "kg_stream_group_abort: null stream");
	for (std::unique_ptr<SeedGroup> &sg : s->groups) {
		std::lock_guard<std::mutex> lk(sg->mu);
		sg->aborted = true;
		sg->cv.notify_all();
	}
	return KG_OK;
}

int kg_stream_fetch_reads(kg_stream *s, int lane, uint8_t *enc, int64_t *read_off)
{
	if (!s || lane < 0 || lane >= (int)s->lanes.size() || !read_off) return fail(KG_ERR_ARG, "kg_stream_fetch_reads: bad argument");
	Lane &l = s->lanes[(size_t)lane];
	if (!l.have_batch) return fail(KG_ERR_ARG, "kg_stream_fetch_reads: no parsed batch in lane %d", lane);
	HIP_TRY(hipSetDevice(s->ix->device));
	HIP_TRY(kgi_sync(l.ws));
	HIP_TRY(hipMemcpy(read_off, l.ws->d_read_off, 8 * (size_t)(l.parsed.n_reads + 1), hipMemcpyDeviceToHost));
	if (enc && l.parsed.n_bases > 0) HIP_TRY(hipMemcpy(enc, l.ws->d_enc, (size_t)l.parsed.n_bases, hipMemcpyDeviceToHost));
	return KG_OK;
}

int kg_stream_fetch(kg_stream *s, int lane, int64_t first, int64_t count)
{
	if (!s || lane < 0 || lane >= (int)s->lanes.size()) return fail(KG_ERR_ARG, "kg_stream_fetch: bad lane");
	Lane &l = s->lanes[(size_t)lane];
	if (first < 0 || count < 0 || first + count > l.mapped_reads || !l.d_records) return fail(KG_ERR_ARG, "kg_stream_fetch: reads [%lld, %lld) are not of the lane's mapped batch (%lld reads)", (long long)first, (long long)(first + count), (long long)l.mapped_reads);
	if (count == 0) return KG_OK;
	kg_workspace *ws = l.ws;
	HIP_TRY(hipSetDevice(ws->ix->device));
	hipStream_t st = ws->stream;
	int64_t *tot = l.h_meta + FQM_WORDS;
	HIP_TRY(hipMemcpyAsync(l.h_records + first, l.d_records + first, sizeof(kg_aln_record) * (size_t)count, hipMemcpyDeviceToHost, st));
	HIP_TRY(hipMemcpyAsync(l.h_cand_off + first, ws->d_cand_off + first, 8 * (size_t)(count + 1), hipMemcpyDeviceToHost, st));
	HIP_TRY(hipMemcpyAsync(&tot[18], ws->d_cseed_off + first, 8, hipMemcpyDeviceToHost, st));
	HIP_TRY(hipMemcpyAsync(&tot[19], ws->d_cseed_off + first + count, 8, hipMemcpyDeviceToHost, st));
	HIP_TRY(kgi_sync(ws));
	const int64_t c0 = l.h_cand_off[first], c1 = l.h_cand_off[first + count], s0 = tot[18], s1 = tot[19];
	if (c0 < 0 || c1 < c0 || c1 > l.h_cand_capacity || s0 < 0 || s1 < s0 || s1 > l.h_cand_capacity) return fail(KG_ERR_NO_DEVICE, "kg_stream_fetch: the batch's candidate offsets are not what kg_stream_map left");
	if (c1 > c0) HIP_TRY(hipMemcpyAsync(l.h_cands + c0, ws->d_dense_cands + c0, sizeof(kg_candidate) * (size_t)(c1 - c0), hipMemcpyDeviceToHost, st));
	if (s1 > s0) HIP_TRY(hipMemcpyAsync(l.h_cand_seeds + s0, ws->d_dense_seeds + s0, sizeof(kg_seed) * (size_t)(s1 - s0), hipMemcpyDeviceToHost, st));
	HIP_TRY(kgi_sync(ws));
	return KG_OK;
}

int kg_stream_timing(kg_stream *s, kg_stream_timing_t *out, int reset)
{
	if (!s || !out) return fail(KG_ERR_ARG, "kg_stream_timing: null argument");
	std::lock_guard<std::mutex> lk(s->mu);
	*out = s->total;
	if (reset) s->total = kg_stream_timing_t{};
	return KG_OK;
}

}
```

kart_amd/csrc/host/knobs.inc:

```
struct Knob { const char *name, *kind, *where, *what; };
static const Knob kKnobs[] = {
	{"KART_AMD_VERBOSE", "D", "host", "per-stage timers of the run on stdout (lane threads, device stages, writer, shards)"},
	{"KART_AMD_SA", "T", "host", "index mode: auto (default) | full | compact | wide | dense4 | dense8 | sampled (kg_index_load's sa_mode)"},
	{"KART_AMD_BATCH_READS", "T", "host", "reads per device call of the host reader's path (default 400000; whole 4000-read chunks)"},
	{"KART_AMD_STREAM_READS", "T", "host", "reads per batch of a device-stream lane (default 1120000)"},
	{"KART_AMD_STREAM_LANES", "T", "host", "lanes of the device stream (default: from the thread count, 8 at -t 16)"},
	{"KART_AMD_SEED_GROUP", "T", "host", "lanes whose batches are seeded by ONE search launch (default 4; 0: every lane seeds its own)"},
	{"KART_AMD_READER_THREADS", "T", "host", "threads of the host FASTQ reader (default (t + 1) / 2)"},
	{"KART_AMD_WRITER_THREADS", "T", "host", "threads copying text into the output file's mapping"},
	{"KART_AMD_PWRITE_THREADS", "T", "host", "of those, how many use pwrite() instead of the mapping (default 1 from 4 writer threads on)"},
	{"KART_AMD_WRITER_MODE", "A", "host", "0 a mapping per chunk, 1 windows unmapped once written (default), 2 windows + MADV_POPULATE_WRITE, 3 windows kept until the end"},
	{"KART_AMD_OUT_WINDOW_MB", "T", "host", "megabytes of the output file one shared mapping (window) of the writers covers (default 1024)"},
	{"KART_AMD_UNMAP_CPUS", "T", "host", "where the thread that unmaps written windows runs: io (the writers' CPUs, default) | lanes"},
	{"KART_AMD_WORKER_NICE", "T", "host", "nice value of the worker pool (default 5: the lane threads come first)"},
	{"KART_AMD_IO_CPUS", "T", "host", "CPU list the reader / writer threads are pinned to"},
	{"KART_AMD_LANE_CPUS", "T", "host", "CPU list the lane threads are pinned to"},
	{"KART_AMD_PREALLOC", "A", "host", "fallocate() the output ahead of the writers"},
	{"KART_AMD_NO_PREALLOC", "A", "host", "... and its off switch"},
	{"KART_AMD_NO_MMAP", "A", "host", "read plain FASTQ through getline() instead of the file's mapping"},
	{"KART_AMD_NO_MMAP_OUT", "A", "host", "write the output with pwrite() only"},
	{"KART_AMD_NO_PREAD", "A", "host", "fill the lanes' staging buffers by memcpy from the mapping instead of pread()"},
	{"KART_AMD_NO_PREFETCH", "D", "host", "the host reader's look-ahead on the main thread (profiling)"},
	{"KART_AMD_NO_BGZF", "A", "host", "inflate BGZF input as one gzip stream"},
	{"KART_AMD_NO_GZ_STREAM", "A", "host", "gz libraries through the host's gz reader (line index, views) instead of the device's FASTQ-in / SAM-out stream"},
	{"KART_AMD_GZ_NO_THP", "A", "host", "no transparent huge pages for the growing block a gz library is inflated into"},
	{"KART_AMD_GZ_AHEAD_MB", "T", "host", "megabytes of inflated text a gz library's thread may be ahead of the device stream (3072)"},
	{"KART_AMD_NO_PGZ", "A", "host", "ordinary gzip input through one gzread() stream per file instead of the several-thread reader"},
	{"KART_AMD_PGZ_CHUNK_KB", "T", "host", "compressed kilobytes per thread and round of the several-thread gzip reader (4096)"},
	{"KART_AMD_PGZ_MIN_KB", "T", "host", "smallest gzip file (compressed kilobytes) the several-thread reader takes (1024)"},
	{"KART_AMD_PGZ_DEBUG", "D", "host", "per-round timings of the several-thread gzip reader on stderr"},
	{"KART_AMD_NO_STREAM", "A", "host", "no device stream: the host parses FASTQ and prints SAM"},
	{"KART_AMD_FETCH_ALL", "A", "host", "the device stream copies every record and candidate of a batch back, not only those of the chunks the host asks for"},
	{"KART_AMD_HOST_ALIGN", "A", "host", "the per-read report on the host's workers (rounds 1-2)"},
	{"KART_AMD_HOST_LONG", "A", "host", "the -pacbio report on the host's workers (round 4)"},
	{"KART_AMD_HOST_FRAGMENTS", "A", "host", "fragment pairs planned by the host instead of kg_fragments_batch"},
	{"KART_AMD_FINISH_STRINGS", "A", "host", "the host's report pass 2 from gapped strings instead of op strings (rounds 2-3)"},
	{"KART_AMD_LONG_NO_OVERLAP", "A", "host", "-pacbio: one workspace, report and next seeding one after the other"},
	{"KART_AMD_PACBIO_CHUNKS", "T", "host", "-pacbio: chunks of the first batch"},
	{"KART_AMD_PACBIO_MAX_CHUNKS", "T", "host", "-pacbio: chunks of a full batch (batches double up to it)"},
	{"KART_AMD_FRAG_SLICE", "T", "host", "-pacbio on the host: fragment pairs per kg_fragments_batch call"},
	{"KART_AMD_FRAG_DEPTH", "T", "host", "... and how many such calls are in flight (1..3)"},
	{"KART_AMD_NO_EAGER_PARTS", "A", "host", "-parts shards hold their text back until the totals in front of them are known"},
	{"KART_AMD_NO_FILE_TURNS", "A", "host", "shards writing one file do not take turns at it"},
	{"KART_AMD_SHARD_TIMEOUT", "T", "host", "seconds a shard waits for another before it gives the run up (default 3600)"},
	{"KART_AMD_MEM_RESERVE_MB", "T", "host", "memory left to others when the output lives in tmpfs (default 512)"},
	{"KART_AMD_UNSET_FLAG", "D", "host", "what a FLAG the reference never assigns prints as (default 0; the tests use 1 << 20)"},
	{"KART_AMD_BACKTRACE", "D", "host", "kh_open installs a SIGSEGV / SIGABRT handler that prints the frames as library offsets"},
	{"KART_AMD_CHECK_ALIGN", "D", "host", "every read mapped on the host as well, device records compared with the host's text"},
	{"KART_AMD_TINY_WORKSPACE", "D", "host", "start with a workspace far too small (exercises growth while results are being read)"},
	{"KART_AMD_OUTPUT_NULL", "M", "host", "the run's text goes to /dev/null (bench.py: gpu_pipeline_value)"},
	{"KG_AUTO_COMPACT", "T", "index", "KG_SA_AUTO never takes the wide index (several processes are going to share the device)"},
	{"KG_QMER", "T", "index", "q of the q-mer table (8..16; default round(log4(2L)), one less in the compact index)"},
	{"KG_NO_QTAB", "A", "index", "no q-mer table: every search starts step by step"},
	{"KG_NO_PLANES2", "A", "index", "no two-step rank planes"},
	{"KG_NO_PLANES3", "A", "index", "no three-step rank planes"},
	{"KG_NO_DIRECT", "A", "index", "single-suffix searches are not finished against the text"},
	{"KG_FORCE_U64", "D", "index", "the 64-bit instantiations on a small index (tests)"},
	{"KG_SEARCH_BLOCKS_PER_CU", "T", "seed", "blocks of search_kernel per CU (default 6, at most 8)"},
	{"KG_FUSED_PACK", "A", "seed", "experiment: no pack pre-pass, the search reads raw codes"},
	{"KG_SORT_READS", "A", "seed", "experiment: reads drawn in the order of their first 16 bases"},
	{"KG_NO_SEGMENTS", "A", "seed", "SensitiveMode: one walk per read instead of walks from every segment start"},
	{"KG_SEG_LEN", "T", "seed", "SensitiveMode: segment length (default 512, at least 128)"},
	{"KG_SPIN_SYNC", "A", "stream", "hipStreamSynchronize instead of the blocking event wait"},
	{"KG_GROUP_NO_TURNS", "A", "stream", "the lanes of a seeding group start their stages at once"},
	{"KG_GROUP_TURN_EARLY", "A", "stream", "a lane passes its group's turn on before its copies back"},
	{"KG_STREAM_CHECKSUM", "M", "stream", "the SAM text of every batch summed on the device (kg_stream_timing_t::text_checksum)"},
	{"KG_ALN_NO_TRIVIAL", "A", "align", "no aln_trivial_kernel: every pair takes the general kernels"},
	{"KG_ALN_INLINE", "A", "align", "a candidate whose alignments are all at most 8 x 8 makes them in its planning lane (measured slower: off by default)"},
	{"KG_ALN_FINISH_LANES", "A", "align", "the finish pass gives a candidate to a lane (rounds 2-5) instead of to a group of eight"},
	{"KG_ALN_FINISH_G16", "A", "align", "the finish pass gives a candidate to sixteen lanes instead of eight"},
	{"KG_ALN_FINISH_WAVE", "A", "align", "the finish pass gives a candidate to a whole wave instead of to a group of eight lanes"},
	{"KG_ALN_PLAN_GROUP", "A", "align", "pass 1 of the report by groups of eight lanes (aln_plan_group_kernel) instead of a candidate per lane"},
	{"KG_ALN_PAIR_HEAVY", "T", "align", "pairs with more candidate pairs (n1 x n2) than this are paired by the whole wave (32)"},
	{"KG_ALN_NO_HEAVY", "A", "align", "pairs with many candidates stay in their lane's loop instead of being the whole wave's"},
	{"KG_ALN_NO_FAST", "A", "align", "no aln_plan_fast_kernel (and no aln_trivial_kernel): every candidate takes aln_plan_kernel"},
	{"KG_ALN_NO_BINS", "A", "align", "aln_plan_kernel takes the candidates in their own order"},
	{"KG_RESCUE_SCAN", "A", "align", "the rescue kernel walks every diagonal of its window (rounds 2-3)"},
	{"KG_NW_NO_TIERS", "A", "align", "the wave-per-pair NW kernel in one tier"},
	{"KG_DBG_NO_PARTITION", "D", "align", "fragments that need the 8-mer partition go back to the host"},
	{"KG_DBG_SPILL_CAPACITY", "D", "align", "the spill list behaves as if it were this short (tests)"},
	{"KG_DBG_JOB_CAPACITY", "D", "align", "the NW job list likewise"},
	{"KG_DBG_OPS_CAPACITY", "D", "align", "the op-byte pool likewise"},
	{"KG_FRAG_NO_FAST_PAIRS", "A", "long", "IdentifyNormalPairs of a fragment on lane 0 only"},
	{"KG_FRAG_TWO_TIERS", "A", "long", "the partition kernel in two launch tiers"},
	{"KG_FRAG_PROF", "D", "long", "wave cycles per phase of the partition kernel"},
	{"KG_LONG_DEBUG", "D", "long", "dump of one read's long-read report"},
	{"KG_LONG_DEBUG_JOBS", "D", "long", "dump of the long-read report's NW jobs"},
	{"KG_LONG_DEBUG_STATUS", "D", "long", "fragment statuses of the long-read report"},
};
```

kart_amd/csrc/stream_kernels.hip:

```cpp
#include "stream_kernels.hpp"

#include <hipcub/hipcub.hpp>

#include <algorithm>

namespace kg {

namespace {

__device__ __forceinline__ uint32_t eq_mask4(uint32_t x, uint32_t pat)
{
	uint32_t t = x ^ pat;
	uint32_t z = ~(((t & 0x7F7F7F7Fu) + 0x7F7F7F7Fu) | t | 0x7F7F7F7Fu);
	return ((z >> 7) & 1u) | ((z >> 14) & 2u) | ((z >> 21) & 4u) | ((z >> 28) & 8u);
}

__device__ __forceinline__ uint32_t newline_mask16(const FqWindow &w, int64_t p, bool &nul)
{
	nul = false;
	if (p >= w.end || p + 16 <= w.begin) return 0;
	const uint4 v = *reinterpret_cast<const uint4 *>(w.text + p);
	uint32_t nl = eq_mask4(v.x, 0x0A0A0A0Au) | (eq_mask4(v.y, 0x0A0A0A0Au) << 4) | (eq_mask4(v.z, 0x0A0A0A0Au) << 8) | (eq_mask4(v.w, 0x0A0A0A0Au) << 12);
	uint32_t z = eq_mask4(v.x, 0u) | (eq_mask4(v.y, 0u) << 4) | (eq_mask4(v.z, 0u) << 8) | (eq_mask4(v.w, 0u) << 12);
	int lo = (int)(w.begin > p ? w.begin - p : 0), hi = (int)(w.end - p < 16 ? w.end - p : 16);
// ... 708 lines not shown
	return bam_block_bytes(t.name_len, lseq) + 4 * bam_cigar_ops(rec) + bam_tag_bytes(t.rlen - rec.score) + bam_tag_bytes(rec.score) + bam_tag_bytes(rec.sub_score);
}

__device__ __forceinline__ int bam_reg2bin(int64_t beg, int64_t end)
{
	--end;
	if (beg >> 14 == end >> 14) return (int)(((1 << 15) - 1) / 7 + (beg >> 14));
	if (beg >> 17 == end >> 17) return (int)(((1 << 12) - 1) / 7 + (beg >> 17));
	if (beg >> 20 == end >> 20) return (int)(((1 << 9) - 1) / 7 + (beg >> 20));
	if (beg >> 23 == end >> 23) return (int)(((1 << 6) - 1) / 7 + (beg >> 23));
	if (beg >> 26 == end >> 26) return (int)(((1 << 3) - 1) / 7 + (beg >> 26));
	return 0;
}

__device__ __forceinline__ void bam_build(const ReadText &t, const kg_aln_record &rec, int lseq, uint32_t *H, uint32_t *C, uint8_t *T, int &nC, int &nT)
{
	const bool mapped = rec.kind == KG_ALN_MAPPED;
	int ops = 0;
	int64_t ref_len = 0;
	uint8_t *q = T;
	if (mapped) {
		uint32_t num = 0;
		for (int i = 0; i < rec.cigar_len; ++i) {
			const char ch = rec.cigar[i];
			if (ch >= '0' && ch <= '9') { num = num * 10u + (uint32_t)(ch - '0'); continue; }
			const int op = bam_cigar_op(ch);
			if (op >= 0 && ops < kBamC / 4) {
				C[ops++] = num << 4 | (uint32_t)op;
				if (op == 0 || op == 2 || op == 3 || op == 7 || op == 8) ref_len += num;
			}
			num = 0;
		}
		q = bam_put_tag(q, 'N', 'M', t.rlen - rec.score);
		q = bam_put_tag(q, 'A', 'S', rec.score);
		q = bam_put_tag(q, 'X', 'S', rec.sub_score);
	} else {
		q = bam_put_tag(q, 'A', 'S', 0);
		q = bam_put_tag(q, 'X', 'S', 0);
	}
	nC = 4 * ops;
	nT = bam_qual_breaks(t) ? 0 : (int)(q - T);
	const int64_t pos = mapped ? rec.pos - 1 : -1;
	const int bin = bam_reg2bin(pos, pos + (ref_len > 0 ? ref_len : 1));
	const bool mate = mapped && rec.has_mate;
	H[0] = (uint32_t)(bam_block_bytes(t.name_len, lseq) + nC + nT - 4);
	H[1] = mapped ? (uint32_t)rec.chr : 0xFFFFFFFFu;
	H[2] = (uint32_t)pos;
	H[3] = (uint32_t)((t.name_len + 1) & 255) | (uint32_t)((mapped ? rec.mapq : 0) & 255) << 8 | (uint32_t)(bin & 0xFFFF) << 16;
	H[4] = (uint32_t)(ops & 0xFFFF) | (uint32_t)(rec.flag & 0xFFFF) << 16;
	H[5] = (uint32_t)lseq;
	H[6] = mate ? (uint32_t)rec.chr : 0xFFFFFFFFu;
	H[7] = mate ? (uint32_t)(rec.mate_pos - 1) : 0xFFFFFFFFu;
	H[8] = mate ? (uint32_t)rec.tlen : 0u;
}

__device__ __forceinline__ uint32_t bam_code4(uint32_t c)
{
	const uint32_t i = (c & 0xDFu) - 0x41u;
	if (i < 16u) return (uint32_t)(0xFFF3FCFFB4FFD2E1ull >> (4u * i)) & 15u;
	if (i < 26u) return (uint32_t)(0xFAF97F865Full >> (4u * (i - 16u))) & 15u;
	return c == '=' ? 0u : 15u;
}

__device__ __forceinline__ uint32_t bam_pack8(uint64_t x)
{
	uint32_t o = 0;
#pragma unroll
	for (int j = 0; j < 4; ++j) {
		const uint32_t hi = bam_code4((uint32_t)(x >> (16 * j)) & 255u), lo = bam_code4((uint32_t)(x >> (16 * j + 8)) & 255u);
		o |= (hi << 4 | lo) << (8 * j);
	}
	return o;
}

__device__ __forceinline__ uint64_t bam_qual8(uint64_t x)
{
	const uint64_t H = 0x8080808080808080ull;
	return ((x | H) - 0x2121212121212121ull) ^ (~x & H);
}

__device__ __forceinline__ bool has_tab8(uint64_t x)
{
	const uint64_t t = x ^ 0x0909090909090909ull;
	return ((t - 0x0101010101010101ull) & ~t & 0x8080808080808080ull) != 0;
}

__device__ __forceinline__ uint32_t bam_shown(const uint8_t *seq, int lseq, bool flip, int i)
{
	return flip ? comp_char(seq[lseq - 1 - i]) : seq[i];
}

__device__ __forceinline__ uint8_t *bam_copy_record(uint8_t *__restrict__ p, int lane, const uint8_t *H, const uint8_t *__restrict__ name, int name_len, const uint8_t *C, int nC,
                                                    const uint8_t *__restrict__ seq, int lseq, bool flip, const uint8_t *__restrict__ qual, int qlen, bool qrev, const uint8_t *T, int nT)
{
	if (lane < kBamCore) p[lane] = H[lane];
	p += kBamCore;
	for (int k = lane; k < name_len; k += 64) p[k] = name[k];
	p += name_len;
	if (lane == 0) *p = 0;
	p += 1;
	for (int k = lane; k < nC; k += 64) p[k] = C[k];
	p += nC;
	const int nb = (lseq + 1) >> 1;
	for (int k = lane; k < nb; k += 64) {
		const uint32_t hi = bam_code4(bam_shown(seq, lseq, flip, 2 * k)), lo = 2 * k + 1 < lseq ? bam_code4(bam_shown(seq, lseq, flip, 2 * k + 1)) : 0u;
		p[k] = (uint8_t)(hi << 4 | lo);
	}
	p += nb;
	bool fill = qlen != lseq || (lseq == 1 && qual[0] == '*') || (qlen > 0 && qual[qlen - 1] == '\n');
	if (!fill) {
		bool tab = false;
		for (int k = lane; k < qlen; k += 64) tab = tab || qual[k] == '\t';
		fill = __any(tab ? 1 : 0) != 0;
	}
	for (int k = lane; k < lseq; k += 64) p[k] = fill ? (uint8_t)0xFF : (uint8_t)((qrev ? qual[lseq - 1 - k] : qual[k]) - 33);
	p += lseq;
	if (lane < nT) p[lane] = T[lane];
	return p + nT;
}

}

__global__ __launch_bounds__(256) void bam_size_kernel(SamArgs a)
{
	for (int64_t r = (int64_t)blockIdx.x * blockDim.x + threadIdx.x; r < a.n_reads; r += (int64_t)gridDim.x * blockDim.x) {
		const kg_aln_record &first = a.records[r];
		int n = 0;
		if (first.kind == KG_ALN_HOST) {
			a.host_list[atomicAdd(&a.ctl[0], 1ull)] = (int32_t)r;
		} else {
			const ReadText t = read_text(a, r);
			for (int64_t at = r; at >= 0; at = a.records[at].next) n += bam_record_size(t, a.records[at], bam_lseq(a, r, t.rlen, a.records[at]));
		}
		a.sam_len[r] = n;
	}
	if (blockIdx.x == 0 && threadIdx.x == 0) a.sam_len[a.n_reads] = 0;
}

__global__ __launch_bounds__(64) void bam_format_kernel(SamArgs a)
{
	__shared__ __attribute__((aligned(16))) uint8_t str[64 * kBamSlot];
	__shared__ BamDesc desc[64];
	__shared__ int chain_len[2];
	__shared__ int chunk_pre[65];
	__shared__ int tab_seen[65];
	const int lane = threadIdx.x;
	const int64_t n_groups = (a.n_reads + 63) >> 6;
	for (int64_t g = blockIdx.x; g < n_groups; g += gridDim.x) {
		{
			const int64_t r = (g << 6) + lane;
			BamDesc d;
			d.flags = 0; d.lseq = 0; d.name_len = 0; d.nC = 0; d.nT = 0;
			tab_seen[lane] = 0;
			if (lane == 0) tab_seen[64] = 0;
			if (r < a.n_reads) {
				const kg_aln_record &rec = a.records[r];
				const int kind = rec.kind;
				if (kind == KG_ALN_UNMAPPED || kind == KG_ALN_MAPPED || (kind != KG_ALN_HOST && rec.next >= 0)) {
					const ReadText t = read_text(a, r);
					const int64_t o0 = a.sam_off[r], o1 = a.sam_off[r + 1];
					const int lseq = bam_lseq(a, r, t.rlen, rec);
					d.name = t.name; d.qual = t.qual; d.seq = a.enc + a.read_off[r];
					d.out = a.sam + o0;
					d.room = (int32_t)(o1 - o0);
					d.name_len = (int16_t)t.name_len; d.lseq = (int16_t)lseq;
					const bool flip = kind == KG_ALN_MAPPED && rec.flip;
					int nC = 0, nT = 0;
					const bool wide = t.rlen > 32000 || t.name_len > 32000 || o1 > a.sam_capacity;
					const bool chained = rec.next >= 0 || wide || (kind != KG_ALN_UNMAPPED && kind != KG_ALN_MAPPED);
					uint8_t *S = str + lane * kBamSlot;
					if (!chained) bam_build(t, rec, lseq, reinterpret_cast<uint32_t *>(S), reinterpret_cast<uint32_t *>(S + kBamH), S + kBamH + kBamC, nC, nT);
					d.nC = (uint8_t)nC; d.nT = (uint8_t)nT;
					const bool qfill = t.qlen != lseq || (lseq == 1 && t.qual[0] == '*') || bam_qual_breaks(t);
					d.flags = (uint8_t)(1 | (flip ? 2 : 0) | (flip != t.held_reversed ? 4 : 0) | (chained ? 8 : 0) | (qfill ? 16 : 0));
				}
			}
			desc[lane] = d;
		}
		__syncthreads();
		{
			const BamDesc d = desc[lane];
			if ((d.flags & 1) && !(d.flags & 8)) {
				const uint8_t *S = str + lane * kBamSlot;
				uint8_t *p = d.out;
				const uint8_t *const end = d.out + d.room;
				uint8_t *const bases = d.out + kBamCore + d.name_len + 1 + d.nC;
				p = lane_copy(p, bases, S, kBamCore);
				p = lane_copy(p, bases, d.name, d.name_len);
				*p++ = 0;
				p = lane_copy(p, bases, S + kBamH, d.nC);
				p += ((d.lseq + 1) >> 1) + d.lseq;
				p = lane_copy(p, end, S + kBamH + kBamC, d.nT);
				if (p != end) atomicAdd(&a.ctl[1], 1ull);
			}
		}
		{
			const BamDesc &dm = desc[lane];
			const bool on = (dm.flags & 1) && !(dm.flags & 8);
			const int mine = on ? ((((dm.lseq + 1) >> 1) + 15) >> 4) + ((dm.lseq + 15) >> 4) : 0;
			const int incl = wave_inclusive_scan(mine);
			if (lane == 0) chunk_pre[0] = 0;
			chunk_pre[lane + 1] = incl;
		}
		__syncthreads();
		{
			const int total = chunk_pre[64];
			int line = 0;
			for (int idx = lane; idx < total; idx += 64) {
				while (idx >= chunk_pre[line + 1]) ++line;
				const BamDesc &d = desc[line];
				const int c = idx - chunk_pre[line];
				const int lseq = d.lseq, nb = (lseq + 1) >> 1;
				const int n_seq = (nb + 15) >> 4;
				uint8_t *const base = d.out + kBamCore + d.name_len + 1 + d.nC;
				if (c < n_seq) {
					const bool flip = (d.flags & 2) != 0;
					uint8_t *dst = base + (c << 4);
					const int b0 = c << 5;
					if (b0 + 32 <= lseq) {
						uint64_t w0, w1, w2, w3;
						if (flip) {
							const SamU128 lo = *reinterpret_cast<const SamU128 *>(d.seq + lseq - 32 - b0), hi = *reinterpret_cast<const SamU128 *>(d.seq + lseq - 16 - b0);
							w0 = comp8(__builtin_bswap64(hi.hi)); w1 = comp8(__builtin_bswap64(hi.lo));
							w2 = comp8(__builtin_bswap64(lo.hi)); w3 = comp8(__builtin_bswap64(lo.lo));
						} else {
							const SamU128 lo = *reinterpret_cast<const SamU128 *>(d.seq + b0), hi = *reinterpret_cast<const SamU128 *>(d.seq + b0 + 16);
							w0 = lo.lo; w1 = lo.hi; w2 = hi.lo; w3 = hi.hi;
						}
						SamU128 o;
						o.lo = (uint64_t)bam_pack8(w0) | (uint64_t)bam_pack8(w1) << 32;
						o.hi = (uint64_t)bam_pack8(w2) | (uint64_t)bam_pack8(w3) << 32;
						*reinterpret_cast<SamU128 *>(dst) = o;
					} else {
						for (int k = c << 4; k < nb; ++k) {
							const uint32_t hi = bam_code4(bam_shown(d.seq, lseq, flip, 2 * k)), lo = 2 * k + 1 < lseq ? bam_code4(bam_shown(d.seq, lseq, flip, 2 * k + 1)) : 0u;
							base[k] = (uint8_t)(hi << 4 | lo);
						}
					}
				} else {
					const int off = (c - n_seq) << 4;
					uint8_t *dst = base + nb + off;
					const bool rev = (d.flags & 4) != 0, fill = (d.flags & 16) != 0;
					if (off + 16 <= lseq) {
						SamU128 v;
						v.lo = v.hi = ~0ull;
						if (!fill) {
							v = *reinterpret_cast<const SamU128 *>(rev ? d.qual + lseq - 16 - off : d.qual + off);
							if (has_tab8(v.lo) || has_tab8(v.hi)) { tab_seen[line] = 1; tab_seen[64] = 1; }
							if (rev) { const uint64_t lo = __builtin_bswap64(v.hi), hi = __builtin_bswap64(v.lo); v.lo = lo; v.hi = hi; }
							v.lo = bam_qual8(v.lo); v.hi = bam_qual8(v.hi);
						}
						*reinterpret_cast<SamU128 *>(dst) = v;
					} else {
						for (int k = off; k < lseq; ++k) {
							const uint8_t b = fill ? (uint8_t)0 : rev ? d.qual[lseq - 1 - k] : d.qual[k];
							if (!fill && b == '\t') { tab_seen[line] = 1; tab_seen[64] = 1; }
							dst[k - off] = fill ? (uint8_t)0xFF : (uint8_t)(b - 33);
						}
					}
				}
			}
		}
		__syncthreads();
		if (tab_seen[64]) {
			for (int i = 0; i < 64; ++i) {
				if (!tab_seen[i]) continue;
				const BamDesc &d = desc[i];
				uint8_t *q = d.out + kBamCore + d.name_len + 1 + d.nC + ((d.lseq + 1) >> 1);
				for (int k = lane; k < d.lseq; k += 64) q[k] = 0xFF;
			}
		}
		for (int i = 0; i < 64; ++i) {
			if (!(desc[i].flags & 1) || !(desc[i].flags & 8)) continue;
			const int64_t r = (g << 6) + i;
			const ReadText t = read_text(a, r);
			const uint8_t *const seq = a.enc + a.read_off[r];
			uint8_t *p = a.sam + a.sam_off[r];
			const int64_t room = a.sam_off[r + 1];
			if (room > a.sam_capacity) { if (lane == 0) atomicAdd(&a.ctl[1], 1ull); continue; }
			uint8_t *S = str + i * kBamSlot;
			for (int64_t at = r; at >= 0; at = a.records[at].next) {
				const kg_aln_record &rec = a.records[at];
				if (rec.kind != KG_ALN_UNMAPPED && rec.kind != KG_ALN_MAPPED) continue;
				const int lseq = bam_lseq(a, r, t.rlen, rec);
				__syncthreads();
				if (lane == 0) bam_build(t, rec, lseq, reinterpret_cast<uint32_t *>(S), reinterpret_cast<uint32_t *>(S + kBamH), S + kBamH + kBamC, chain_len[0], chain_len[1]);
				__syncthreads();
				const bool flip = rec.kind == KG_ALN_MAPPED && rec.flip;
				p = bam_copy_record(p, lane, S, t.name, t.name_len, S + kBamH, chain_len[0], seq, lseq, flip, t.qual, t.qlen, flip != t.held_reversed, S + kBamH + kBamC, chain_len[1]);
			}
			if (lane == 0 && (int64_t)(p - a.sam) != room) atomicAdd(&a.ctl[1], 1ull);
		}
		__syncthreads();
	}
}

__global__ void sam_reset_kernel(SamArgs a)
{
	if (threadIdx.x < 4) a.ctl[threadIdx.x] = 0;
}

__global__ __launch_bounds__(256) void sam_checksum_kernel(SamArgs a)
{
	const int64_t bytes = a.sam_off[a.n_reads];
	const int64_t n16 = bytes >> 4;
	unsigned long long sum = 0, lines = 0;
	const uint4 *src = reinterpret_cast<const uint4 *>(a.sam);
	for (int64_t i = (int64_t)blockIdx.x * blockDim.x + threadIdx.x; i < n16; i += (int64_t)gridDim.x * blockDim.x) {
		const uint4 v = src[i];
		const uint32_t w[4] = {v.x, v.y, v.z, v.w};
#pragma unroll
		for (int k = 0; k < 4; ++k) {
			sum += (w[k] & 255u) + ((w[k] >> 8) & 255u) + ((w[k] >> 16) & 255u) + (w[k] >> 24);
			const uint32_t x = w[k] ^ 0x0A0A0A0Au;
			lines += __popc(((x - 0x01010101u) & ~x) & 0x80808080u);
		}
	}
	if (blockIdx.x == 0 && threadIdx.x < (bytes & 15)) {
		const uint8_t c = a.sam[(n16 << 4) + threadIdx.x];
		sum += c; lines += c == 10 ? 1 : 0;
	}
	for (int off = 32; off > 0; off >>= 1) { sum += __shfl_down(sum, off); lines += __shfl_down(lines, off); }
	if ((threadIdx.x & 63) == 0 && (sum | lines)) { atomicAdd(&a.ctl[2], sum); atomicAdd(&a.ctl[3], lines); }
}

namespace {

struct Widen32 {
	__host__ __device__ __forceinline__ int64_t operator()(const int32_t &x) const { return (int64_t)x; }
};
using Wide32Iter = hipcub::TransformInputIterator<int64_t, Widen32, const int32_t *>;

inline int grid_of(int64_t items, int block, int max_blocks)
{
	int64_t g = (items + block - 1) / block;
	if (g < 1) g = 1;
	if (g > max_blocks) g = max_blocks;
	return (int)g;
}

}

size_t fq_scan_temp_bytes(int64_t max_items)
{
	size_t b1 = 0, b2 = 0;
	Wide32Iter it((const int32_t *)nullptr, Widen32());
	(void)hipcub::DeviceScan::ExclusiveSum(nullptr, b1, it, (int64_t *)nullptr, (int)max_items);
	(void)hipcub::DeviceScan::ExclusiveSum(nullptr, b2, (const int32_t *)nullptr, (int32_t *)nullptr, (int)max_items);
	return b1 > b2 ? b1 : b2;
}

size_t fa_scan_temp_bytes(int64_t max_lines)
{
	size_t b = 0;
	(void)hipcub::DeviceScan::ExclusiveSum(nullptr, b, (const uint64_t *)nullptr, (uint64_t *)nullptr, (int)(max_lines + 1));
	return b;
}

hipError_t launch_fq_parse(const FqArgs &a, void *scan_temp, size_t scan_temp_bytes, int n_cu, hipStream_t stream)
{
	hipError_t e;
	kt_begin(KT_FQ_PARSE, stream);
	hipLaunchKernelGGL(fq_reset_kernel, dim3(grid_of(a.max_reads + 1, 256, n_cu * 8)), dim3(256), 0, stream, a);
	for (int f = 0; f < (a.two_files ? 2 : 1); ++f) {
		const FqWindow &w = a.w[f];
		const int64_t ta = w.begin & ~(int64_t)15;
		const int64_t n_tiles = w.end > ta ? (w.end - ta + kFqTile - 1) / kFqTile : 0;
		hipLaunchKernelGGL(fq_count_kernel, dim3(grid_of(n_tiles, 1, n_cu * 64)), dim3(256), 0, stream, a, f, n_tiles);
		size_t tb = scan_temp_bytes;
		if ((e = hipcub::DeviceScan::ExclusiveSum(scan_temp, tb, (const int32_t *)w.tile_lines, w.tile_lines, (int)(n_tiles + 1), stream)) != hipSuccess) return e;
		hipLaunchKernelGGL(fq_index_kernel, dim3(grid_of(n_tiles, 1, n_cu * 64)), dim3(256), 0, stream, a, f, n_tiles);
		if (a.fasta) {
			const int64_t n_scan = std::min<int64_t>(w.line_capacity, w.end - w.begin + 1);
			hipLaunchKernelGGL(fa_line_kernel, dim3(grid_of(n_scan + 1, 256, n_cu * 16)), dim3(256), 0, stream, a, f, n_scan);
			tb = scan_temp_bytes;
			if ((e = hipcub::DeviceScan::ExclusiveSum(scan_temp, tb, (const uint64_t *)w.line_acc, w.line_acc, (int)(n_scan + 1), stream)) != hipSuccess) return e;
			hipLaunchKernelGGL(fa_head_kernel, dim3(grid_of(n_scan, 256, n_cu * 16)), dim3(256), 0, stream, a, f);
			hipLaunchKernelGGL(fa_record_kernel, dim3(grid_of(std::min<int64_t>(w.rec_capacity, n_scan), 256, n_cu * 16)), dim3(256), 0, stream, a, f);
		} else
		hipLaunchKernelGGL(fq_record_kernel, dim3(grid_of(w.line_capacity / 4, 256, n_cu * 16)), dim3(256), 0, stream, a, f);
	}
	size_t tb = scan_temp_bytes;
	Wide32Iter it(a.read_len, Widen32());
	if ((e = hipcub::DeviceScan::ExclusiveSum(scan_temp, tb, it, a.read_off, (int)(a.max_reads + 1), stream)) != hipSuccess) return e;
	hipLaunchKernelGGL(fq_plan_kernel, dim3(1), dim3(64), 0, stream, a);
	kt_end(KT_FQ_PARSE, stream);
	return hipGetLastError();
}

hipError_t launch_fq_materialise(const FqArgs &a, int n_cu, hipStream_t stream)
{
	if (a.n_reads <= 0) return hipSuccess;
	kt_begin(KT_FQ_MATERIALISE, stream);
	if (a.fasta) hipLaunchKernelGGL(fa_materialise_kernel, dim3(grid_of(a.n_reads * 8, 256, n_cu * 16)), dim3(256), 0, stream, a);
	else hipLaunchKernelGGL(fq_materialise_kernel, dim3(grid_of(a.n_reads * 8, 256, n_cu * 16)), dim3(256), 0, stream, a);
	kt_end(KT_FQ_MATERIALISE, stream);
	return hipGetLastError();
}

__global__ __launch_bounds__(256) void group_publish_kernel(const int64_t *local_off, int64_t n, int64_t slots, int64_t enc_base, int64_t *g_off, int32_t *g_len)
{
	const int64_t stride = (int64_t)gridDim.x * blockDim.x;
	for (int64_t i = (int64_t)blockIdx.x * blockDim.x + threadIdx.x; i < slots; i += stride) {
		const int64_t at = local_off[i < n ? i : n];
		g_off[i] = enc_base + at;
		g_len[i] = i < n ? (int32_t)(local_off[i + 1] - at) : 0;
	}
}

__global__ __launch_bounds__(256) void group_rebase_kernel(const int64_t *g_seed_off, int64_t n, int64_t first, int64_t *seed_off)
{
	const int64_t stride = (int64_t)gridDim.x * blockDim.x;
	for (int64_t i = (int64_t)blockIdx.x * blockDim.x + threadIdx.x; i <= n; i += stride) seed_off[i] = g_seed_off[i] - first;
}

hipError_t launch_group_publish(const int64_t *local_off, int64_t n, int64_t slots, int64_t enc_base, int64_t *g_off, int32_t *g_len, int n_cu, hipStream_t stream)
{
	hipLaunchKernelGGL(group_publish_kernel, dim3(grid_of(slots, 256, n_cu * 8)), dim3(256), 0, stream, local_off, n, slots, enc_base, g_off, g_len);
	return hipGetLastError();
}

hipError_t launch_group_rebase(const int64_t *g_seed_off, int64_t n, int64_t first, int64_t *seed_off, int n_cu, hipStream_t stream)
{
	hipLaunchKernelGGL(group_rebase_kernel, dim3(grid_of(n + 1, 256, n_cu * 8)), dim3(256), 0, stream, g_seed_off, n, first, seed_off);
	return hipGetLastError();
}

hipError_t launch_sam_size(const SamArgs &a, void *scan_temp, size_t scan_temp_bytes, int n_cu, hipStream_t stream)
{
	kt_begin(KT_SAM_SIZE, stream);
	hipLaunchKernelGGL(sam_reset_kernel, dim3(1), dim3(64), 0, stream, a);
	hipLaunchKernelGGL(sam_size_kernel, dim3(grid_of(a.n_reads, 256, n_cu * 16)), dim3(256), 0, stream, a);
	size_t tb = scan_temp_bytes;
	Wide32Iter it(a.sam_len, Widen32());
	hipError_t e = hipcub::DeviceScan::ExclusiveSum(scan_temp, tb, it, a.sam_off, (int)(a.n_reads + 1), stream);
	if (e != hipSuccess) return e;
	kt_end(KT_SAM_SIZE, stream);
	return hipGetLastError();
}

hipError_t launch_sam_format(const SamArgs &a, int n_cu, hipStream_t stream)
{
	if (a.n_reads <= 0) return hipSuccess;
	kt_begin(KT_SAM_FORMAT, stream);
	hipLaunchKernelGGL(sam_format_kernel, dim3(grid_of((a.n_reads + 63) / 64, 1, n_cu * 64)), dim3(64), 0, stream, a);
	kt_end(KT_SAM_FORMAT, stream);
	return hipGetLastError();
}

hipError_t launch_bam_size(const SamArgs &a, void *scan_temp, size_t scan_temp_bytes, int n_cu, hipStream_t stream)
{
	kt_begin(KT_SAM_SIZE, stream);
	hipLaunchKernelGGL(sam_reset_kernel, dim3(1), dim3(64), 0, stream, a);
	hipLaunchKernelGGL(bam_size_kernel, dim3(grid_of(a.n_reads, 256, n_cu * 16)), dim3(256), 0, stream, a);
	size_t tb = scan_temp_bytes;
	Wide32Iter it(a.sam_len, Widen32());
	hipError_t e = hipcub::DeviceScan::ExclusiveSum(scan_temp, tb, it, a.sam_off, (int)(a.n_reads + 1), stream);
	if (e != hipSuccess) return e;
	kt_end(KT_SAM_SIZE, stream);
	return hipGetLastError();
}

hipError_t launch_bam_format(const SamArgs &a, int n_cu, hipStream_t stream)
{
	if (a.n_reads <= 0) return hipSuccess;
	kt_begin(KT_SAM_FORMAT, stream);
	hipLaunchKernelGGL(bam_format_kernel, dim3(grid_of((a.n_reads + 63) / 64, 1, n_cu * 64)), dim3(64), 0, stream, a);
	kt_end(KT_SAM_FORMAT, stream);
	return hipGetLastError();
}

hipError_t launch_sam_checksum(const SamArgs &a, int n_cu, hipStream_t stream)
{
	if (a.n_reads <= 0) return hipSuccess;
	hipLaunchKernelGGL(sam_checksum_kernel, dim3(n_cu * 8), dim3(256), 0, stream, a);
	return hipGetLastError();
}

}
```

Measured before the change: 49.66 million.

## Overlap parse, format and copy-back across lanes with shared group streams

Lanes in a seeding group now share the group workspace's stream for compute, and a separate input stream and copy stream are created per stream object. Parsing and uploads run on the input stream, and device-to-host copies run on the copy stream behind an event. SAM sizing and formatting are launched speculatively in one go, and the group turn is released before the host waits; if the output buffer was too small, the lane reallocates and redoes the step. This removes a host sync between sizing and formatting and lets one lane's copy-back overlap the next lane's compute, at the cost of more cross-stream event dependencies and an occasional redo.

```diff
diff --git a/kart_amd/csrc/abi.hip b/kart_amd/csrc/abi.hip
--- a/kart_amd/csrc/abi.hip
+++ b/kart_amd/csrc/abi.hip
@@ -424,6 +424,11 @@
 
 int kg_workspace_create(kg_index *ix, int64_t max_reads, int64_t max_bases, kg_workspace **out)
 {
+	return kgi_workspace_create(ix, max_reads, max_bases, nullptr, out);
+}
+
+int kgi_workspace_create(kg_index *ix, int64_t max_reads, int64_t max_bases, hipStream_t borrow, kg_workspace **out)
+{
 	if (!ix || !out || max_reads <= 0 || max_bases <= 0) return fail(KG_ERR_ARG, "kg_workspace_create: bad argument");
 	*out = nullptr;
 	HIP_TRY(hipSetDevice(ix->device));
@@ -443,7 +448,8 @@
 		HIP_TRY(hipMalloc((void **)&ws->d_sort_keys, 16 * (size_t)max_reads + 64));
 		HIP_TRY(hipMalloc(&ws->d_sort_temp, ws->sort_bytes ? ws->sort_bytes : 256));
 	}
-	HIP_TRY(hipStreamCreateWithFlags(&ws->stream, hipStreamNonBlocking));
+	if (borrow) { ws->stream = borrow; ws->stream_borrowed = true; }
+	else HIP_TRY(hipStreamCreateWithFlags(&ws->stream, hipStreamNonBlocking));
 	HIP_TRY(hipMemsetAsync(ws->d_ctl, 0, 8 * kCtlWords, ws->stream));
 	HIP_TRY(hipHostMalloc((void **)&ws->h_small, 8 * 16, hipHostMallocDefault));
 	*out = ws.release();
@@ -454,7 +460,8 @@
 {
 	if (!ws) return;
 	(void)hipSetDevice(ws->ix->device);
-	if (ws->stream) { (void)hipStreamSynchronize(ws->stream); (void)hipStreamDestroy(ws->stream); }
+	if (ws->stream) (void)hipStreamSynchronize(ws->stream);
+	if (ws->stream && !ws->stream_borrowed) (void)hipStreamDestroy(ws->stream);
 	kgi_long_release(ws);
 	for (int i = 0; i < kg_workspace::kRing; ++i) {
 		if (ws->ring_cands[i]) (void)hipHostFree(ws->ring_cands[i]);
diff --git a/kart_amd/csrc/abi_internal.hpp b/kart_amd/csrc/abi_internal.hpp
--- a/kart_amd/csrc/abi_internal.hpp
+++ b/kart_amd/csrc/abi_internal.hpp
@@ -142,6 +142,7 @@
 	int chunk_capacity = 0;
 	unsigned long long *d_aln_ctl = nullptr;
 	hipStream_t stream = nullptr;
+	bool stream_borrowed = false;
 	hipEvent_t sync_ev = nullptr;
 	unsigned long long *h_small = nullptr;
 	bool profiling = false;
@@ -152,6 +153,7 @@
 
 extern "C" {
 KG_INTERNAL hipError_t kgi_sync(kg_workspace *ws);
+KG_INTERNAL int kgi_workspace_create(kg_index *ix, int64_t max_reads, int64_t max_bases, hipStream_t borrow, kg_workspace **out);
 KG_INTERNAL int kgi_seed_resident(kg_workspace *ws, int mode, int min_seed_len, int occ_thr, int64_t n_reads, int64_t n_bases, int64_t *total_out);
 KG_INTERNAL int kgi_seed_group(kg_workspace *ws, int mode, int min_seed_len, int occ_thr, int n_seg, int64_t stride, const int64_t *counts, int64_t *seed_base);
 KG_INTERNAL int kgi_chain_resident(kg_workspace *ws, int pacbio, int max_gaps, int64_t totals[2]);
diff --git a/kart_amd/csrc/abi_stream.hip b/kart_amd/csrc/abi_stream.hip
--- a/kart_amd/csrc/abi_stream.hip
+++ b/kart_amd/csrc/abi_stream.hip
@@ -1,5 +1,6 @@
 #include "abi_internal.hpp"
 #include "stream_kernels.hpp"
+#include "stream_sizes.hpp"
 
 #include <algorithm>
 #include <chrono>
@@ -52,6 +53,7 @@
 	bool fasta = false;
 	hipEvent_t ev[8] = {nullptr, nullptr, nullptr, nullptr, nullptr, nullptr, nullptr, nullptr};
 	hipEvent_t ev_parsed = nullptr;
+	hipEvent_t ev_wait = nullptr;
 };
 
 struct SeedGroup {
@@ -71,17 +73,28 @@
 	bool aborted = false;
 	int order[kMaxSeedSegments] = {0};
 	int n_order = 0, turn = 0;
+	bool busy = false;
 };
 
 struct GroupTurn {
 	SeedGroup *sg = nullptr;
-	bool held = false;
+	bool held = false, in_order = false;
 	bool acquire(SeedGroup &g, int j)
 	{
 		sg = &g;
 		std::unique_lock<std::mutex> lk(g.mu);
-		g.cv.wait(lk, [&]() { return g.aborted || (g.turn < g.n_order && g.order[g.turn] == j); });
+		g.cv.wait(lk, [&]() { return g.aborted || (!g.busy && g.turn < g.n_order && g.order[g.turn] == j); });
 		held = !g.aborted;
+		if (held) { g.busy = true; in_order = true; }
+		return held;
+	}
+	bool acquire_again(SeedGroup &g)
+	{
+		sg = &g;
+		std::unique_lock<std::mutex> lk(g.mu);
+		g.cv.wait(lk, [&]() { return g.aborted || !g.busy; });
+		held = !g.aborted;
+		if (held) { g.busy = true; in_order = false; }
 		return held;
 	}
 	void release()
@@ -89,7 +102,8 @@
 		if (!held) return;
 		held = false;
 		std::lock_guard<std::mutex> lk(sg->mu);
-		sg->turn++;
+		sg->busy = false;
+		if (in_order) sg->turn++;
 		sg->cv.notify_all();
 	}
 	~GroupTurn() { release(); }
@@ -103,6 +117,7 @@
 	int64_t text_capacity = 0, line_capacity = 0, rec_capacity = 0;
 	std::vector<Lane> lanes;
 	std::vector<std::unique_ptr<SeedGroup>> groups;
+	hipStream_t in_stream = nullptr, copy_stream = nullptr;
 	uint8_t *d_chr_names = nullptr;
 	int32_t *d_chr_name_off = nullptr;
 	int min_seed_len = 13;
@@ -119,6 +134,7 @@
 {
 	if (l.ws && l.ws->enc_borrowed) l.ws->d_enc = nullptr;
 	if (l.ev_parsed) (void)hipEventDestroy(l.ev_parsed);
+	if (l.ev_wait) (void)hipEventDestroy(l.ev_wait);
 	if (l.ws) kg_workspace_destroy(l.ws);
 	for (int f = 0; f < 2; ++f) {
 		if (l.d_text[f]) (void)hipFree(l.d_text[f]);
@@ -160,6 +176,23 @@
 int64_t out_capacity(const kg_stream_config &cfg, int format)
 {
 	return 2 * cfg.max_window + (format == KG_STREAM_FORMAT_BAM ? 144 : 64) * cfg.max_reads + 4096;
+}
+
+hipStream_t in_stream_of(const kg_stream *s, const Lane &l) { return s->in_stream ? s->in_stream : l.ws->stream; }
+hipStream_t copy_stream_of(const kg_stream *s, const Lane &l) { return s->copy_stream ? s->copy_stream : l.ws->stream; }
+
+hipError_t wait_behind(Lane &l, hipStream_t st)
+{
+	hipError_t e = hipEventRecord(l.ev_wait, st);
+	return e != hipSuccess ? e : hipEventSynchronize(l.ev_wait);
+}
+
+hipError_t quiesce(const kg_stream *s, const Lane &l)
+{
+	hipError_t e = hipStreamSynchronize(l.ws->stream);
+	if (e == hipSuccess && s->in_stream) e = hipStreamSynchronize(s->in_stream);
+	if (e == hipSuccess && s->copy_stream) e = hipStreamSynchronize(s->copy_stream);
+	return e;
 }
 
 float elapsed(hipEvent_t a, hipEvent_t b)
@@ -224,9 +257,13 @@
 		HIP_TRY(hipHostMalloc((void **)&sg->h_ctl, 8 * kCtlWords, hipHostMallocDefault));
 		(void)kg_workspace_set_profiling(gw, 1);
 	}
+	if (group) {
+		HIP_TRY(hipStreamCreateWithFlags(&s->in_stream, hipStreamNonBlocking));
+		HIP_TRY(hipStreamCreateWithFlags(&s->copy_stream, hipStreamNonBlocking));
+	}
 	for (size_t li = 0; li < s->lanes.size(); ++li) {
 		Lane &l = s->lanes[li];
-		int rc = kg_workspace_create(ix, n + 8, cfg->max_window + 4096, &l.ws);
+		int rc = kgi_workspace_create(ix, n + 8, cfg->max_window + 4096, group ? s->groups[li / (size_t)group]->ws->stream : nullptr, &l.ws);
 		if (rc != KG_OK) return rc;
 		kg_workspace *ws = l.ws;
 		if (group) {
@@ -268,6 +305,7 @@
 		l.record_capacity = n + n / 4 + 4096;
 		HIP_TRY(hipHostMalloc((void **)&l.h_records, sizeof(kg_aln_record) * (size_t)l.record_capacity, hipHostMallocDefault));
 		for (hipEvent_t &e : l.ev) HIP_TRY(hipEventCreate(&e));
+		HIP_TRY(hipEventCreateWithFlags(&l.ev_wait, hipEventBlockingSync | hipEventDisableTiming));
 	}
 	HIP_TRY(hipDeviceSynchronize());
 	*out = s.release();
@@ -284,6 +322,8 @@
 		if (sg->ws) kg_workspace_destroy(sg->ws);
 		if (sg->h_ctl) (void)hipHostFree(sg->h_ctl);
 	}
+	for (hipStream_t st : {s->in_stream, s->copy_stream})
+		if (st) { (void)hipStreamSynchronize(st); (void)hipStreamDestroy(st); }
 	if (s->d_chr_names) (void)hipFree(s->d_chr_names);
 	if (s->d_chr_name_off) (void)hipFree(s->d_chr_name_off);
 	delete s;
@@ -297,13 +337,13 @@
 	const int64_t want = out_capacity(s->cfg, format);
 	for (Lane &l : s->lanes) {
 		if (l.d_sam_capacity < want) {
-			HIP_TRY(hipStreamSynchronize(l.ws->stream));
+			HIP_TRY(quiesce(s, l));
 			HIP_TRY(hipFree(l.d_sam)); l.d_sam = nullptr; l.d_sam_capacity = 0;
 			HIP_TRY(hipMalloc((void **)&l.d_sam, (size_t)want));
 			l.d_sam_capacity = want;
 		}
 		if (l.h_sam_capacity < want) {
-			HIP_TRY(hipStreamSynchronize(l.ws->stream));
+			HIP_TRY(quiesce(s, l));
 			HIP_TRY(hipHostFree(l.h_sam)); l.h_sam = nullptr; l.h_sam_capacity = 0;
 			HIP_TRY(hipHostMalloc((void **)&l.h_sam, (size_t)want, hipHostMallocDefault));
 			l.h_sam_capacity = want;
@@ -323,7 +363,7 @@
 		const int64_t rec_capacity = s->line_capacity / 2 + 1;
 		for (Lane &l : s->lanes) {
 			if (s->fasta_sized) break;
-			HIP_TRY(hipStreamSynchronize(l.ws->stream));
+			HIP_TRY(quiesce(s, l));
 			for (int f = 0; f < 2; ++f) {
 				uint32_t *wider = nullptr;
 				HIP_TRY(hipMalloc((void **)&wider, 4 * 6 * (size_t)rec_capacity));
@@ -335,7 +375,7 @@
 				HIP_TRY(hipMemset(l.d_rec_line[f], 0, 4 * (size_t)(rec_capacity + 1)));
 			}
 			if (l.scan_bytes < want_scan) {
-				HIP_TRY(hipStreamSynchronize(l.ws->stream));
+				HIP_TRY(quiesce(s, l));
 				HIP_TRY(hipFree(l.d_scan)); l.d_scan = nullptr; l.scan_bytes = 0;
 				HIP_TRY(hipMalloc(&l.d_scan, want_scan));
 				l.scan_bytes = want_scan;
@@ -361,7 +401,7 @@
 	if (to == from) return KG_OK;
 	Lane &l = s->lanes[(size_t)lane];
 	HIP_TRY(hipSetDevice(s->ix->device));
-	HIP_TRY(hipMemcpyAsync(l.d_text[file] + from, l.h_text[file] + from, (size_t)(to - from), hipMemcpyHostToDevice, l.ws->stream));
+	HIP_TRY(hipMemcpyAsync(l.d_text[file] + from, l.h_text[file] + from, (size_t)(to - from), hipMemcpyHostToDevice, in_stream_of(s, l)));
 	return KG_OK;
 }
 
@@ -395,12 +435,12 @@
 	a.read_off = ws->d_read_off;
 	a.enc = ws->d_enc;
 	a.n_reads = 0;
-	hipStream_t st = ws->stream;
+	hipStream_t st = in_stream_of(s, l);
 	KtUse kt_use(ws->profiling ? &ws->kt : nullptr);
 	HIP_TRY(hipEventRecord(l.ev[0], st));
 	HIP_TRY(launch_fq_parse(a, l.d_scan, l.scan_bytes, s->ix->n_cu, st));
 	HIP_TRY(hipMemcpyAsync(l.h_meta, l.d_meta, 8 * FQM_WORDS, hipMemcpyDeviceToHost, st));
-	HIP_TRY(kgi_sync(ws));
+	HIP_TRY(st == ws->stream ? kgi_sync(ws) : wait_behind(l, st));
 	kg_stream_parsed &p = l.parsed;
 	p.n_reads = l.h_meta[FQM_READS]; p.n_chunks = l.h_meta[FQM_CHUNKS]; p.n_bases = l.h_meta[FQM_BASES];
 	p.used[0] = l.h_meta[FQM_USED0]; p.used[1] = w->two_files ? l.h_meta[FQM_USED1] : 0;
@@ -539,9 +579,9 @@
 	double group_useful = 0;
 	int rc;
 	GroupTurn turn;
+	static const bool no_turns = getenv("KG_GROUP_NO_TURNS") != nullptr;
 	if (grouped) {
 		rc = group_seed(s, lane, n, l.parsed.n_bases, &n_seeds, &group_leader, &group_search_ms, &group_useful);
-		static const bool no_turns = getenv("KG_GROUP_NO_TURNS") != nullptr;
 		SeedGroup &sg = *s->groups[(size_t)lane / (size_t)s->cfg.seed_group];
 		if (rc == KG_OK && !no_turns && !turn.acquire(sg, lane - sg.first)) rc = fail(KG_ERR_ARG, "kg_stream_map: the stream's seeding groups were aborted");
 		if (rc != KG_OK) {
@@ -580,25 +620,43 @@
 	q.sam_len = l.d_sam_len; q.sam_off = l.d_sam_off; q.sam = l.d_sam; q.sam_capacity = l.d_sam_capacity;
 	q.host_list = l.d_host_list; q.ctl = l.d_sam_ctl;
 	const bool bam = s->format == KG_STREAM_FORMAT_BAM;
-	HIP_TRY(bam ? launch_bam_size(q, l.d_scan, l.scan_bytes, ix->n_cu, st) : launch_sam_size(q, l.d_scan, l.scan_bytes, ix->n_cu, st));
+	const bool checksum = getenv("KG_STREAM_CHECKSUM") != nullptr;
 	int64_t *tot = l.h_meta + FQM_WORDS;
-	HIP_TRY(hipMemcpyAsync(&tot[0], l.d_sam_off + n, 8, hipMemcpyDeviceToHost, st));
-	HIP_TRY(hipMemcpyAsync(&tot[1], l.d_sam_ctl, 8, hipMemcpyDeviceToHost, st));
-	HIP_TRY(hipMemcpyAsync(&tot[3], ws->d_aln_ctl + 7, 8, hipMemcpyDeviceToHost, st));
-	HIP_TRY(kgi_sync(ws));
+	auto size_and_format = [&]() -> int {
+		HIP_TRY(bam ? launch_bam_size(q, l.d_scan, l.scan_bytes, ix->n_cu, st) : launch_sam_size(q, l.d_scan, l.scan_bytes, ix->n_cu, st));
+		HIP_TRY(hipMemcpyAsync(&tot[0], l.d_sam_off + n, 8, hipMemcpyDeviceToHost, st));
+		HIP_TRY(hipMemcpyAsync(&tot[1], l.d_sam_ctl, 8, hipMemcpyDeviceToHost, st));
+		HIP_TRY(hipMemcpyAsync(&tot[3], ws->d_aln_ctl + 7, 8, hipMemcpyDeviceToHost, st));
+		HIP_TRY(bam ? launch_bam_format(q, ix->n_cu, st) : launch_sam_format(q, ix->n_cu, st));
+		if (checksum) HIP_TRY(launch_sam_checksum(q, ix->n_cu, st));
+		HIP_TRY(hipEventRecord(l.ev[5], st));
+		HIP_TRY(hipEventRecord(l.ev_wait, st));
+		return KG_OK;
+	};
+	rc = size_and_format();
+	if (rc != KG_OK) return rc;
+	turn.release();
+	HIP_TRY(hipEventSynchronize(l.ev_wait));
+	const kg::OutGrowth grow = kg::out_growth(tot[0], l.d_sam_capacity, l.h_sam_capacity);
+	if (grow.h_capacity != l.h_sam_capacity) {
+		HIP_TRY(hipHostFree(l.h_sam)); l.h_sam = nullptr; l.h_sam_capacity = 0;
+		HIP_TRY(hipHostMalloc((void **)&l.h_sam, (size_t)grow.h_capacity, hipHostMallocDefault));
+		l.h_sam_capacity = grow.h_capacity;
+	}
+	if (grow.redo) {
+		HIP_TRY(hipFree(l.d_sam)); l.d_sam = nullptr; l.d_sam_capacity = 0;
+		HIP_TRY(hipMalloc((void **)&l.d_sam, (size_t)grow.d_capacity));
+		l.d_sam_capacity = grow.d_capacity;
+		q.sam = l.d_sam; q.sam_capacity = l.d_sam_capacity;
+		if (grouped && !no_turns && !turn.acquire_again(*s->groups[(size_t)lane / (size_t)s->cfg.seed_group])) return fail(KG_ERR_ARG, "kg_stream_map: the stream's seeding groups were aborted");
+		rc = size_and_format();
+		if (rc != KG_OK) return rc;
+		turn.release();
+		HIP_TRY(hipEventSynchronize(l.ev_wait));
+		if (tot[0] > l.d_sam_capacity) return fail(KG_ERR_NO_DEVICE, "kg_stream_map: the batch's text grew from one sizing to the next");
+	}
 	const int64_t sam_bytes = tot[0], n_host = tot[1];
 	const int64_t extra = prm->multi_hit ? std::min<int64_t>(tot[3], a.extra_capacity) : 0;
-	if (sam_bytes > l.d_sam_capacity) {
-		HIP_TRY(hipFree(l.d_sam)); l.d_sam = nullptr;
-		l.d_sam_capacity = sam_bytes + sam_bytes / 4;
-		HIP_TRY(hipMalloc((void **)&l.d_sam, (size_t)l.d_sam_capacity));
-		q.sam = l.d_sam; q.sam_capacity = l.d_sam_capacity;
-	}
-	if (sam_bytes > l.h_sam_capacity) {
-		HIP_TRY(hipHostFree(l.h_sam)); l.h_sam = nullptr;
-		l.h_sam_capacity = sam_bytes + sam_bytes / 4;
-		HIP_TRY(hipHostMalloc((void **)&l.h_sam, (size_t)l.h_sam_capacity, hipHostMallocDefault));
-	}
 	const int64_t cand_need = std::max(totals[0], totals[1]);
 	if (cand_need > l.h_cand_capacity) {
 		if (l.h_cands) HIP_TRY(hipHostFree(l.h_cands));
@@ -608,31 +666,29 @@
 		HIP_TRY(hipHostMalloc((void **)&l.h_cands, sizeof(kg_candidate) * (size_t)l.h_cand_capacity, hipHostMallocDefault));
 		HIP_TRY(hipHostMalloc((void **)&l.h_cand_seeds, sizeof(kg_seed) * (size_t)l.h_cand_capacity, hipHostMallocDefault));
 	}
-	HIP_TRY(bam ? launch_bam_format(q, ix->n_cu, st) : launch_sam_format(q, ix->n_cu, st));
-	const bool checksum = getenv("KG_STREAM_CHECKSUM") != nullptr;
-	if (checksum) HIP_TRY(launch_sam_checksum(q, ix->n_cu, st));
-	HIP_TRY(hipEventRecord(l.ev[5], st));
-	static const bool turn_early = getenv("KG_GROUP_TURN_EARLY") != nullptr;
-	if (turn_early) turn.release();
-	if (sam_bytes > 0) HIP_TRY(hipMemcpyAsync(l.h_sam, l.d_sam, (size_t)sam_bytes, hipMemcpyDeviceToHost, st));
-	HIP_TRY(hipMemcpyAsync(l.h_sam_off, l.d_sam_off, 8 * (size_t)(n + 1), hipMemcpyDeviceToHost, st));
+	hipStream_t cst = copy_stream_of(s, l);
+	if (cst != st) HIP_TRY(hipStreamWaitEvent(cst, l.ev[5], 0));
+	HIP_TRY(hipEventRecord(l.ev[7], cst));
+	if (sam_bytes > 0) HIP_TRY(hipMemcpyAsync(l.h_sam, l.d_sam, (size_t)sam_bytes, hipMemcpyDeviceToHost, cst));
+	HIP_TRY(hipMemcpyAsync(l.h_sam_off, l.d_sam_off, 8 * (size_t)(n + 1), hipMemcpyDeviceToHost, cst));
 	const bool all = prm->fetch_all != 0;
 	l.mapped_reads = n; l.d_records = a.records;
-	if (all) HIP_TRY(hipMemcpyAsync(l.h_records, a.records, sizeof(kg_aln_record) * (size_t)(n + extra), hipMemcpyDeviceToHost, st));
-	else if (extra > 0) HIP_TRY(hipMemcpyAsync(l.h_records + n, a.records + n, sizeof(kg_aln_record) * (size_t)extra, hipMemcpyDeviceToHost, st));
-	HIP_TRY(hipMemcpyAsync(l.h_chunk_stats, ws->d_chunk_stats, sizeof(kg_chunk_stats) * (size_t)n_chunks, hipMemcpyDeviceToHost, st));
-	if (all) HIP_TRY(hipMemcpyAsync(l.h_cand_off, ws->d_cand_off, 8 * (size_t)(n + 1), hipMemcpyDeviceToHost, st));
-	if (n_host > 0) HIP_TRY(hipMemcpyAsync(l.h_host_list, l.d_host_list, 4 * (size_t)n_host, hipMemcpyDeviceToHost, st));
-	if (all && totals[0] > 0) HIP_TRY(hipMemcpyAsync(l.h_cands, ws->d_dense_cands, sizeof(kg_candidate) * (size_t)totals[0], hipMemcpyDeviceToHost, st));
-	if (all && totals[1] > 0) HIP_TRY(hipMemcpyAsync(l.h_cand_seeds, ws->d_dense_seeds, sizeof(kg_seed) * (size_t)totals[1], hipMemcpyDeviceToHost, st));
-	HIP_TRY(hipMemcpyAsync(&tot[2], l.d_sam_ctl + 1, 8, hipMemcpyDeviceToHost, st));
-	HIP_TRY(hipMemcpyAsync(&tot[8], ws->d_aln_ctl, 8 * 7, hipMemcpyDeviceToHost, st));
-	HIP_TRY(hipMemcpyAsync(&tot[15], ws->d_aln_ctl + 32, 8, hipMemcpyDeviceToHost, st));
+	if (all) HIP_TRY(hipMemcpyAsync(l.h_records, a.records, sizeof(kg_aln_record) * (size_t)(n + extra), hipMemcpyDeviceToHost, cst));
+	else if (extra > 0) HIP_TRY(hipMemcpyAsync(l.h_records + n, a.records + n, sizeof(kg_aln_record) * (size_t)extra, hipMemcpyDeviceToHost, cst));
+	HIP_TRY(hipMemcpyAsync(l.h_chunk_stats, ws->d_chunk_stats, sizeof(kg_chunk_stats) * (size_t)n_chunks, hipMemcpyDeviceToHost, cst));
+	if (all) HIP_TRY(hipMemcpyAsync(l.h_cand_off, ws->d_cand_off, 8 * (size_t)(n + 1), hipMemcpyDeviceToHost, cst));
+	if (n_host > 0) HIP_TRY(hipMemcpyAsync(l.h_host_list, l.d_host_list, 4 * (size_t)n_host, hipMemcpyDeviceToHost, cst));
+	if (all && totals[0] > 0) HIP_TRY(hipMemcpyAsync(l.h_cands, ws->d_dense_cands, sizeof(kg_candidate) * (size_t)totals[0], hipMemcpyDeviceToHost, cst));
+	if (all && totals[1] > 0) HIP_TRY(hipMemcpyAsync(l.h_cand_seeds, ws->d_dense_seeds, sizeof(kg_seed) * (size_t)totals[1], hipMemcpyDeviceToHost, cst));
+	HIP_TRY(hipMemcpyAsync(&tot[2], l.d_sam_ctl + 1, 8, hipMemcpyDeviceToHost, cst));
+	HIP_TRY(hipMemcpyAsync(&tot[8], ws->d_aln_ctl, 8 * 7, hipMemcpyDeviceToHost, cst));
+	HIP_TRY(hipMemcpyAsync(&tot[15], ws->d_aln_ctl + 32, 8, hipMemcpyDeviceToHost, cst));
 	tot[16] = tot[17] = 0;
-	if (checksum) HIP_TRY(hipMemcpyAsync(&tot[16], l.d_sam_ctl + 2, 16, hipMemcpyDeviceToHost, st));
-	HIP_TRY(hipMemcpyAsync(&tot[14], ws->d_aln_ctl + 36, 8, hipMemcpyDeviceToHost, st));
-	HIP_TRY(hipEventRecord(l.ev[6], st));
-	HIP_TRY(kgi_sync(ws));
+	if (checksum) HIP_TRY(hipMemcpyAsync(&tot[16], l.d_sam_ctl + 2, 16, hipMemcpyDeviceToHost, cst));
+	HIP_TRY(hipMemcpyAsync(&tot[14], ws->d_aln_ctl + 36, 8, hipMemcpyDeviceToHost, cst));
+	HIP_TRY(hipEventRecord(l.ev[6], cst));
+	HIP_TRY(wait_behind(l, cst));
+	if (in_stream_of(s, l) != st) HIP_TRY(hipEventSynchronize(l.ev[1]));
 	if (tot[2] != 0) return fail(KG_ERR_NO_DEVICE, "kg_stream_map: %lld records were formatted to a size other than the one announced", (long long)tot[2]);
 	std::sort(l.h_host_list, l.h_host_list + n_host);
 	out->n_reads = n; out->n_chunks = n_chunks;
@@ -654,7 +710,7 @@
 		kg_stream_timing_t &t = s->total;
 		t.batches += 1; t.reads += n;
 		t.parse_ms += elapsed(l.ev[0], l.ev[1]); t.seed_ms += elapsed(l.ev[1], l.ev[2]); t.chain_ms += elapsed(l.ev[2], l.ev[3]);
-		t.align_ms += elapsed(l.ev[3], l.ev[4]); t.format_ms += elapsed(l.ev[4], l.ev[5]); t.copy_ms += elapsed(l.ev[5], l.ev[6]);
+		t.align_ms += elapsed(l.ev[3], l.ev[4]); t.format_ms += elapsed(l.ev[4], l.ev[5]); t.copy_ms += elapsed(l.ev[7], l.ev[6]);
 		t.search_kernel_ms += sk; t.search_kernel_launches += (!grouped || group_leader) ? 1 : 0; t.search_useful_bytes += useful;
 		t.text_in_bytes += (double)((l.parsed.used[0] - l.win.begin[0]) + (l.win.two_files ? l.parsed.used[1] - l.win.begin[1] : 0));
 		t.text_out_bytes += (double)sam_bytes;
@@ -684,8 +740,8 @@
 		Lane &l = s->lanes[(size_t)lane];
 		HIP_TRY(hipSetDevice(s->ix->device));
 		HIP_TRY(launch_group_publish(l.ws->d_read_off, 0, sg.stride, (int64_t)j * sg.seg_bases, sg.ws->d_read_off + (int64_t)j * sg.stride, sg.ws->group_read_len + (int64_t)j * sg.stride,
-		                             s->ix->n_cu, l.ws->stream));
-		HIP_TRY(hipEventRecord(l.ev_parsed, l.ws->stream));
+		                             s->ix->n_cu, in_stream_of(s, l)));
+		HIP_TRY(hipEventRecord(l.ev_parsed, in_stream_of(s, l)));
 	}
 	sg.absent_rounds[j] = rounds;
 	if (rounds == 0) sg.aborted = false;
@@ -718,7 +774,7 @@
 	Lane &l = s->lanes[(size_t)lane];
 	if (!l.have_batch) return fail(KG_ERR_ARG, "kg_stream_fetch_reads: no parsed batch in lane %d", lane);
 	HIP_TRY(hipSetDevice(s->ix->device));
-	HIP_TRY(kgi_sync(l.ws));
+	HIP_TRY(hipEventSynchronize(l.ev[1]));
 	HIP_TRY(hipMemcpy(read_off, l.ws->d_read_off, 8 * (size_t)(l.parsed.n_reads + 1), hipMemcpyDeviceToHost));
 	if (enc && l.parsed.n_bases > 0) HIP_TRY(hipMemcpy(enc, l.ws->d_enc, (size_t)l.parsed.n_bases, hipMemcpyDeviceToHost));
 	return KG_OK;
@@ -732,18 +788,18 @@
 	if (count == 0) return KG_OK;
 	kg_workspace *ws = l.ws;
 	HIP_TRY(hipSetDevice(ws->ix->device));
-	hipStream_t st = ws->stream;
+	hipStream_t st = copy_stream_of(s, l);
 	int64_t *tot = l.h_meta + FQM_WORDS;
 	HIP_TRY(hipMemcpyAsync(l.h_records + first, l.d_records + first, sizeof(kg_aln_record) * (size_t)count, hipMemcpyDeviceToHost, st));
 	HIP_TRY(hipMemcpyAsync(l.h_cand_off + first, ws->d_cand_off + first, 8 * (size_t)(count + 1), hipMemcpyDeviceToHost, st));
 	HIP_TRY(hipMemcpyAsync(&tot[18], ws->d_cseed_off + first, 8, hipMemcpyDeviceToHost, st));
 	HIP_TRY(hipMemcpyAsync(&tot[19], ws->d_cseed_off + first + count, 8, hipMemcpyDeviceToHost, st));
-	HIP_TRY(kgi_sync(ws));
+	HIP_TRY(wait_behind(l, st));
 	const int64_t c0 = l.h_cand_off[first], c1 = l.h_cand_off[first + count], s0 = tot[18], s1 = tot[19];
 	if (c0 < 0 || c1 < c0 || c1 > l.h_cand_capacity || s0 < 0 || s1 < s0 || s1 > l.h_cand_capacity) return fail(KG_ERR_NO_DEVICE, "kg_stream_fetch: the batch's candidate offsets are not what kg_stream_map left");
 	if (c1 > c0) HIP_TRY(hipMemcpyAsync(l.h_cands + c0, ws->d_dense_cands + c0, sizeof(kg_candidate) * (size_t)(c1 - c0), hipMemcpyDeviceToHost, st));
 	if (s1 > s0) HIP_TRY(hipMemcpyAsync(l.h_cand_seeds + s0, ws->d_dense_seeds + s0, sizeof(kg_seed) * (size_t)(s1 - s0), hipMemcpyDeviceToHost, st));
-	HIP_TRY(kgi_sync(ws));
+	HIP_TRY(wait_behind(l, st));
 	return KG_OK;
 }
 
diff --git a/kart_amd/csrc/host/knobs.inc b/kart_amd/csrc/host/knobs.inc
--- a/kart_amd/csrc/host/knobs.inc
+++ b/kart_amd/csrc/host/knobs.inc
@@ -63,7 +63,6 @@
 	{"KG_SEG_LEN", "T", "seed", "SensitiveMode: segment length (default 512, at least 128)"},
 	{"KG_SPIN_SYNC", "A", "stream", "hipStreamSynchronize instead of the blocking event wait"},
 	{"KG_GROUP_NO_TURNS", "A", "stream", "the lanes of a seeding group start their stages at once"},
-	{"KG_GROUP_TURN_EARLY", "A", "stream", "a lane passes its group's turn on before its copies back"},
 	{"KG_STREAM_CHECKSUM", "M", "stream", "the SAM text of every batch summed on the device (kg_stream_timing_t::text_checksum)"},
 	{"KG_ALN_NO_TRIVIAL", "A", "align", "no aln_trivial_kernel: every pair takes the general kernels"},
 	{"KG_ALN_INLINE", "A", "align", "a candidate whose alignments are all at most 8 x 8 makes them in its planning lane (measured slower: off by default)"},
diff --git a/kart_amd/csrc/stream_kernels.hip b/kart_amd/csrc/stream_kernels.hip
--- a/kart_amd/csrc/stream_kernels.hip
+++ b/kart_amd/csrc/stream_kernels.hip
@@ -1034,7 +1034,7 @@
 
 __global__ __launch_bounds__(256) void sam_checksum_kernel(SamArgs a)
 {
-	const int64_t bytes = a.sam_off[a.n_reads];
+	const int64_t bytes = a.sam_off[a.n_reads] < a.sam_capacity ? a.sam_off[a.n_reads] : a.sam_capacity;
 	const int64_t n16 = bytes >> 4;
 	unsigned long long sum = 0, lines = 0;
 	const uint4 *src = reinterpret_cast<const uint4 *>(a.sam);
diff --git a/kart_amd/csrc/stream_sizes.hpp b/kart_amd/csrc/stream_sizes.hpp
--- /dev/null
+++ b/kart_amd/csrc/stream_sizes.hpp
@@ -0,0 +1,20 @@
+#pragma once
+#include <cstdint>
+
+namespace kg {
+
+struct OutGrowth {
+	int64_t d_capacity;
+	int64_t h_capacity;
+	bool redo;
+};
+
+inline OutGrowth out_growth(int64_t text_bytes, int64_t d_capacity, int64_t h_capacity)
+{
+	OutGrowth g{d_capacity, h_capacity, false};
+	if (text_bytes > d_capacity) { g.d_capacity = text_bytes + text_bytes / 4; g.redo = true; }
+	if (text_bytes > h_capacity) g.h_capacity = text_bytes + text_bytes / 4;
+	return g;
+}
+
+}
```

Result: slower. 44.12 million (-11.2%).
